# bitlayer-org/tap-stark

Measured on AMD Instinct MI355X. Metric: trace cells/sec (proofs/sec alongside), 2^20x64 BabyBear trace, higher is better.
Workload: dtype u32

## Files before the change

tap-stark_amd/csrc/context.cpp:

```cpp
#include <errno.h>
#include <stdio.h>
#include <time.h>
#include <stdlib.h>
#include "context.hpp"

#include <string.h>

#include "kernels.hpp"

namespace ts {

static bool poison_knob(uint32_t* word) {
    const char* e = getenv("TS_POOL_POISON");
    if (!e || !*e) return false;
    char* end = nullptr;
    errno = 0;
    const unsigned long v = strtoul(e, &end, 0);
    TS_REQUIRE(errno == 0 && end != e && *end == 0 && e[0] != '-' && v <= 0xFFFFFFFFul, TS_ERR_INVALID,
               "TS_POOL_POISON is not a 32-bit word (decimal, 0x hex or 0 octal)");
    *word = (uint32_t)v;
    return true;
}

Context::Context(int dev) : device(dev) {
    pool_debug = getenv("TS_POOL_DEBUG") != nullptr;
    poison_on = poison_knob(&poison_word);
    int count = 0;
    hipError_t e = hipGetDeviceCount(&count);
    if (e != hipSuccess || count == 0)
        throw Error(TS_ERR_HIP, "no HIP device available: the tap-stark HIP path has no CPU fallback");
    TS_REQUIRE(dev >= 0 && dev < count, TS_ERR_INVALID, "device index out of range");
    TS_HIP(hipSetDevice(dev));
    hipDeviceProp_t prop;
    TS_HIP(hipGetDeviceProperties(&prop, dev));
    num_cus = prop.multiProcessorCount;
    max_lds_per_block = prop.sharedMemPerBlock;
    arch_name = prop.gcnArchName;
    arch_name = arch_name.substr(0, arch_name.find(':'));
    TS_HIP(hipStreamCreateWithFlags(&stream, hipStreamNonBlocking));
}

Context::~Context() {
    (void)hipSetDevice(device);
    if (stream) (void)hipStreamSynchronize(stream);
    if (d_twiddle_fwd) (void)hipFree(d_twiddle_fwd);
    if (d_twiddle_inv) (void)hipFree(d_twiddle_inv);
    for (auto& t : scale_tables) (void)hipFree(t.d);
    for (auto& t : sel_tables)
        if (t.d) (void)hipFree(t.d);
    if (d_ticket) (void)hipFree(d_ticket);
    for (auto& kv : free_blocks) (void)hipFree(kv.second);
    for (auto& kv : live_blocks) (void)hipFree(kv.first);
    if (h_pinned) (void)hipHostFree(h_pinned);
    if (h_mailbox) (void)hipHostFree(h_mailbox);
    if (h_mailbox_big) (void)hipHostFree(h_mailbox_big);
    if (h_arena) (void)hipHostFree(h_arena);
    if (stream) (void)hipStreamDestroy(stream);
}

static size_t round_block(size_t bytes) {
    if (bytes < 512) return 512;
    if (bytes < (1u << 20)) {
        size_t r = 512;
        while (r < bytes) r <<= 1;
        return r;
    }
    const size_t g = 1u << 20;
    return (bytes + g - 1) / g * g;
}

void* Context::alloc(size_t bytes) {
    const size_t sz = round_block(bytes);
    auto it = free_blocks.find(sz);
    void* p = nullptr;
    if (it != free_blocks.end()) {
        p = it->second;
        free_blocks.erase(it);
    } else {
        TS_HIP(hipSetDevice(device));
        if (pool_debug) {
            struct timespec ts_;
            clock_gettime(CLOCK_MONOTONIC, &ts_);
            fprintf(stderr, "[ts pool %p t=%.3f ms] hipMalloc %zu KiB (reserved %zu MiB)\n", (void*)this,
                    ts_.tv_sec * 1e3 + ts_.tv_nsec * 1e-6, sz >> 10, bytes_reserved >> 20);
        }
        hipError_t e = hipMalloc(&p, sz);
        if (e != hipSuccess) {
            release_cache();
            e = hipMalloc(&p, sz);
        }
        if (e != hipSuccess) {
            (void)hipGetLastError();
            throw Error(TS_ERR_OOM, "device allocation failed");
        }
        bytes_reserved += sz;
    }
    live_blocks[p] = sz;
    if (poison_on) poison(p, sz);
    return p;
}

void Context::poison(void* p, size_t bytes) {
    TS_HIP(hipSetDevice(device));
    TS_HIP(hipMemsetD32Async((hipDeviceptr_t)p, (int)poison_word, bytes / 4, stream));
    TS_HIP(hipStreamSynchronize(stream));
    poison_fills++;
}

void Context::free(void* p) {
    if (!p) return;
    auto it = live_blocks.find(p);
    if (it == live_blocks.end()) return;
    free_blocks.emplace(it->second, p);
    live_blocks.erase(it);
}

void Context::release_cache() {
    if (stream) (void)hipStreamSynchronize(stream);
    for (auto& kv : free_blocks) {
        (void)hipFree(kv.second);
        bytes_reserved -= kv.first;
    }
    free_blocks.clear();
}

uint32_t* Context::ticket() {
    if (!d_ticket) {
        TS_HIP(hipMalloc((void**)&d_ticket, 64 * 17));
        TS_HIP(hipMemsetAsync(d_ticket, 0, 64 * 17, stream));
    }
    return d_ticket;
}

const void* Context::stage(const void* src, size_t bytes) {
    const size_t need = (bytes + 63) & ~(size_t)63;
    if (need > h_arena_bytes / 2) {
        sync();
        if (h_arena) (void)hipHostFree(h_arena);
        h_arena = nullptr;
        size_t sz = 1 << 20;
        while (sz / 2 < need) sz <<= 1;
        TS_HIP(hipHostMalloc((void**)&h_arena, sz, hipHostMallocDefault));
        h_arena_bytes = sz;
        h_arena_off = 0;
    }
    if (h_arena_off + need > h_arena_bytes) {
        sync();
        h_arena_off = 0;
    }
    void* p = h_arena + h_arena_off;
    memcpy(p, src, bytes);
    h_arena_off += need;
    return p;
}

void Context::sync_point(void* host, size_t bytes) {
    if (replay_mode == 2 && replay_pos < replay_log.size() && replay_log[replay_pos].size() == bytes) {
        memcpy(host, replay_log[replay_pos++].data(), bytes);
        return;
    }
    sync();
    if (replay_mode == 1) replay_log.emplace_back((const char*)host, (const char*)host + bytes);
}
void Context::d2h_point(void* host_dst, const void* dev_src, size_t bytes) {
    if (replay_mode == 2 && replay_pos < replay_log.size() && replay_log[replay_pos].size() == bytes) {
        memcpy(host_dst, replay_log[replay_pos++].data(), bytes);
        return;
    }
    if (bytes) TS_HIP(hipMemcpyAsync(host_dst, dev_src, bytes, hipMemcpyDeviceToHost, stream));
    sync();
    if (replay_mode == 1) replay_log.emplace_back((const char*)host_dst, (const char*)host_dst + bytes);
}

uint32_t* Context::mailbox(size_t words) {
    constexpr size_t WORDS = 16384;
    if (words > WORDS / 4) {
        if (words > h_mailbox_big_words) {
            sync();
            if (h_mailbox_big) (void)hipHostFree(h_mailbox_big);
            h_mailbox_big = nullptr;
            h_mailbox_big_words = 0;
            TS_HIP(hipHostMalloc((void**)&h_mailbox_big, words * 4, hipHostMallocDefault));
            h_mailbox_big_words = words;
        }
        return h_mailbox_big;
    }
    if (!h_mailbox) TS_HIP(hipHostMalloc((void**)&h_mailbox, WORDS * 4, hipHostMallocDefault));
    const size_t need = (words + 15) & ~(size_t)15;
    if (mailbox_off + need > WORDS) mailbox_off = 0;
    uint32_t* p = h_mailbox + mailbox_off;
    mailbox_off += need;
    return p;
}

void* Context::pinned(size_t bytes) {
    if (bytes > h_pinned_bytes) {
        if (h_pinned) {
            sync();
            (void)hipHostFree(h_pinned);
        }
        size_t sz = 1 << 16;
        while (sz < bytes) sz <<= 1;
        TS_HIP(hipHostMalloc(&h_pinned, sz, hipHostMallocDefault));
        h_pinned_bytes = sz;
    }
    return h_pinned;
}

std::map<std::string, std::pair<uint64_t, double>> Context::take_kernel_timings() {
    std::map<std::string, std::pair<uint64_t, double>> out;
    sync();
    for (auto& ev : kernel_events) {
        float ms = 0;
        (void)hipEventElapsedTime(&ms, ev.e0, ev.e1);
        auto& slot = out[ev.name];
        slot.first += 1;
        slot.second += ms;
        (void)hipEventDestroy(ev.e0);
        (void)hipEventDestroy(ev.e1);
    }
    kernel_events.clear();
    return out;
}

void Context::ensure_twiddles(unsigned log_size) {
    if (log_size <= twiddle_log && d_twiddle_fwd) return;
    TS_REQUIRE(log_size <= 27, TS_ERR_INVALID, "two-adicity of BabyBear is 27");
    sync();
    if (d_twiddle_fwd) (void)hipFree(d_twiddle_fwd);
    if (d_twiddle_inv) (void)hipFree(d_twiddle_inv);
    d_twiddle_fwd = d_twiddle_inv = nullptr;
    const size_t n = (size_t)1 << log_size;
    TS_HIP(hipMalloc((void**)&d_twiddle_fwd, n * 4));
    TS_HIP(hipMalloc((void**)&d_twiddle_inv, n * 4));
    if (poison_on) {
        poison(d_twiddle_fwd, n * 4);
        poison(d_twiddle_inv, n * 4);
    }
    twiddle_log = log_size;
    launch_build_twiddles(*this, d_twiddle_fwd, d_twiddle_inv, log_size);
}

}
```

tap-stark_amd/csrc/context.hpp:

```cpp
#pragma once
#include <hip/hip_runtime.h>
#include <stdint.h>

#include <map>
#include <stdexcept>
#include <string>
#include <vector>

#include "bb.hpp"

namespace ts {

struct Error : std::runtime_error {
    int code;
    Error(int c, const std::string& m) : std::runtime_error(m), code(c) {}
};

struct FinalPolyNotConstant : Error {
    explicit FinalPolyNotConstant(const std::string& m) : Error(5 , m) {}
};

enum : int {
    TS_OK = 0,
    TS_ERR_INVALID = 1,
    TS_ERR_HIP = 2,
    TS_ERR_OOM = 3,
    TS_ERR_UNSUPPORTED = 4,
    TS_ERR_INVARIANT = 5,
    TS_ERR_BUFFER = 6,
    TS_ERR_COMM = 7,
};

#define TS_HIP(expr)                                                                        \
    do {                                                                                    \
        hipError_t _e = (expr);                                                             \
        if (_e != hipSuccess)                                                               \
            throw ts::Error(ts::TS_ERR_HIP, std::string(#expr) + ": " + hipGetErrorString(_e)); \
    } while (0)

#define TS_REQUIRE(cond, code, msg)                   \
    do {                                              \
        if (!(cond)) throw ts::Error((code), (msg));  \
    } while (0)

struct Context {
    int device = 0;
    hipStream_t stream = nullptr;
    std::string last_error;
    int num_cus = 256;
    size_t max_lds_per_block = 64 * 1024;
    std::string arch_name;

    std::multimap<size_t, void*> free_blocks;
    std::map<void*, size_t> live_blocks;
    size_t bytes_reserved = 0;
    bool pool_debug = false;
    bool poison_on = false;
    uint32_t poison_word = 0;
    uint64_t poison_fills = 0;
    void poison(void* p, size_t bytes);

    uint32_t* d_twiddle_fwd = nullptr;
    uint32_t* d_twiddle_inv = nullptr;
    unsigned twiddle_log = 0;

    struct ScaleTable {
        unsigned log_n, log_blowup;
        uint32_t shift;
        uint32_t* d;
        size_t words;
        uint64_t last_use;
    };
    std::vector<ScaleTable> scale_tables;
    uint64_t scale_clock = 0;
    struct SelTable {
        uint32_t* d = nullptr;
        unsigned log_n = ~0u, log_qd = ~0u;
        uint32_t shift = 0;
        uint64_t last_use = 0;
    };
    SelTable sel_tables[2];
    uint64_t sel_clock = 0;

    uint32_t* d_ticket = nullptr;
    uint32_t* ticket();

    unsigned lde_pass_mask = 7;

    uint32_t* h_mailbox = nullptr;
    size_t mailbox_off = 0;
    uint32_t* h_mailbox_big = nullptr;
    size_t h_mailbox_big_words = 0;
    uint32_t* mailbox(size_t words);

    void* h_pinned = nullptr;
    size_t h_pinned_bytes = 0;
    char* h_arena = nullptr;
    size_t h_arena_bytes = 0, h_arena_off = 0;
    const void* stage(const void* src, size_t bytes);

    bool timing = false;
    std::vector<std::pair<std::string, float>> stage_ms;

    struct KernelEvent {
        const char* name;
        hipEvent_t e0, e1;
    };
    bool kernel_timing = false;
    std::vector<KernelEvent> kernel_events;
    std::map<std::string, std::pair<uint64_t, double>> take_kernel_timings();

    uint64_t pow_hints_accepted = 0, pow_hints_rejected = 0, pow_host_grinds = 0;
    uint64_t local_quotient_fallbacks = 0;

    explicit Context(int dev);
    ~Context();
    Context(const Context&) = delete;

    void* alloc(size_t bytes);
    void free(void* p);
    template <class T>
    T* alloc_n(size_t n) { return static_cast<T*>(alloc(n * sizeof(T))); }
    void release_cache();

    int replay_mode = 0;
    size_t replay_pos = 0;
    std::vector<std::vector<char>> replay_log;
    void sync_point(void* host, size_t bytes);
    void d2h_point(void* host_dst, const void* dev_src, size_t bytes);
    void* pinned(size_t bytes);
    void ensure_twiddles(unsigned log_size);
    void sync() { TS_HIP(hipStreamSynchronize(stream)); }
};

template <class T>
struct DevBuf {
    Context* ctx = nullptr;
    T* p = nullptr;
    size_t n = 0;
    DevBuf() = default;
    DevBuf(Context* c, size_t count) : ctx(c), p(c->alloc_n<T>(count)), n(count) {}
    DevBuf(const DevBuf&) = delete;
    DevBuf& operator=(const DevBuf&) = delete;
    DevBuf(DevBuf&& o) noexcept : ctx(o.ctx), p(o.p), n(o.n) { o.p = nullptr; }
    DevBuf& operator=(DevBuf&& o) noexcept {
        if (this != &o) {
            reset();
            ctx = o.ctx; p = o.p; n = o.n; o.p = nullptr;
        }
        return *this;
    }
    ~DevBuf() { reset(); }
    void reset() {
        if (p) ctx->free(p);
        p = nullptr;
    }
};

struct KernelTimer {
    Context* ctx;
    Context::KernelEvent ev;
    bool on;
    KernelTimer(Context* c, const char* name) : ctx(c), on(c->kernel_timing) {
        if (on) {
            ev.name = name;
            (void)hipEventCreate(&ev.e0);
            (void)hipEventCreate(&ev.e1);
            (void)hipEventRecord(ev.e0, ctx->stream);
        }
    }
    ~KernelTimer() {
        if (on) {
            (void)hipEventRecord(ev.e1, ctx->stream);
            ctx->kernel_events.push_back(ev);
        }
    }
};

#define TS_LAUNCH_NAMED(ctx, name, kernel, grid, block, lds, ...)                   \
    do {                                                                            \
        ts::KernelTimer _kt(&(ctx), name);                                          \
        hipLaunchKernelGGL(kernel, grid, block, lds, (ctx).stream, __VA_ARGS__);    \
    } while (0)
#define TS_LAUNCH(ctx, kernel, ...) TS_LAUNCH_NAMED(ctx, #kernel, kernel, __VA_ARGS__)

struct StageTimer {
    Context* ctx;
    const char* name;
    hipEvent_t e0 = nullptr, e1 = nullptr;
    StageTimer(Context* c, const char* n) : ctx(c), name(n) {
        if (ctx->timing) {
            (void)hipEventCreate(&e0);
            (void)hipEventCreate(&e1);
            (void)hipEventRecord(e0, ctx->stream);
        }
    }
    ~StageTimer() {
        if (ctx->timing && e0) {
            (void)hipEventRecord(e1, ctx->stream);
            (void)hipEventSynchronize(e1);
            float ms = 0;
            (void)hipEventElapsedTime(&ms, e0, e1);
            ctx->stage_ms.emplace_back(name, ms);
            (void)hipEventDestroy(e0);
            (void)hipEventDestroy(e1);
        }
    }
};

}
```

tap-stark_amd/csrc/host.hpp:

```cpp
#pragma once
#include <stdint.h>

#include <algorithm>
#include <functional>
#include <memory>
#include <vector>

#include "air.hpp"
#include "bb.hpp"
#include "chal_dev.hpp"
#include "context.hpp"
#include "kernels.hpp"

namespace ts {

class BfChallenger {
public:
    enum Permutation { Blake3Permutation = 0, TestReversePermutation = 1 };
    BfChallenger(int permutation, bool sample_ext)
        : permutation_(permutation), sample_ext_(sample_ext) {}

    void observe(uint32_t word);
    void observe_commitment(const uint32_t d[8]);
    uint32_t sample_base();
    Ef sample_ext();
    Ef sample();
    uint64_t sample_bits(unsigned bits);
    bool check_witness(unsigned bits, uint32_t witness);
    uint32_t grind(unsigned bits);
    void export_state(uint32_t out[34]) const;
    void export_dev(DevChallenger& d) const;
    void import_dev(const DevChallenger& d);

private:
    void duplexing();
    uint32_t pop();
    uint32_t state_[16] = {0};
    uint32_t in_[8] = {0};
    int n_in_ = 0;
    uint32_t out_[8] = {0};
    int n_out_ = 0;
    int permutation_;
    bool sample_ext_;
};

struct FriConfig {
    uint32_t log_blowup = 1;
    uint32_t num_queries = 1;
    uint32_t proof_of_work_bits = 0;
    uint32_t blowup() const { return 1u << log_blowup; }
};

struct DeviceMatrix {
    enum Layout { ROW_MAJOR, COL_MAJOR_BITREV };
    DevBuf<uint32_t> buf;
    uint64_t height = 0;
    uint32_t width = 0;
    Layout layout = ROW_MAJOR;
};

struct PcsData {
    std::vector<DevBuf<uint32_t>> lde_storage;
    std::vector<ColMat> ldes;
    unsigned log_height = 0;
    DevBuf<uint32_t> tree;
    DevBuf<const uint32_t*> col_table;
    bool col_table_uploaded = false;
    uint32_t root[8] = {0};
    LeafMats leaf_mats() const;
    LeafMats leaf_mats_with_table(Context& ctx);
};
std::vector<const uint32_t*> column_pointers(const std::vector<ColMat>& ldes, uint64_t height = 0);
bool columns_as_one_matrix(const std::vector<ColMat>& ldes, uint64_t height, uint32_t max_width, ColMat& one);

unsigned log2_strict(uint64_t n);

void mmcs_commit(Context& ctx, PcsData& data);

class TwoAdicFriPcs {
public:
    TwoAdicFriPcs(Context& ctx, FriConfig fri) : ctx_(ctx), fri_(fri) {}
    const FriConfig& fri() const { return fri_; }
    Context& ctx() const { return ctx_; }

    std::unique_ptr<PcsData> commit(std::vector<DeviceMatrix>& evals,
                                    const std::vector<uint32_t>& domain_shifts, bool build_tree = true,
                                    bool keep_row_major = false);

    std::vector<DeviceMatrix> quotient_chunks(const PcsData& trace_data, const AirProgram& air,
                                              const std::vector<uint32_t>& public_values, Ef alpha,
                                              const PcsData* preprocessed = nullptr, const PcsData* aux = nullptr);

    DevBuf<Ef> open_reduce(const PcsData& trace_data, const PcsData& quotient_data, Ef zeta,
                           Ef batch_alpha, std::vector<Ef>& opened_values, const PcsData* preprocessed = nullptr,
                           const PcsData* aux = nullptr);

    struct Slab {
        uint64_t row0 = 0, rows = 0;
        uint32_t beta0 = 0;
    };
    std::vector<DeviceMatrix> quotient_chunks_slab(const ColMat& lde_slab, unsigned log_n, const Slab& slab,
                                                   const AirProgram& air,
                                                   const std::vector<uint32_t>& public_values, Ef alpha,
                                                   uint32_t domain_shift = GENERATOR,
                                                   const ColMat* prep_lde = nullptr, const ColMat* aux_lde = nullptr);
    DevBuf<Ef> open_reduce_slab(const PcsData& trace_data, const PcsData& quotient_data, unsigned log_N,
                                const Slab& slab, Ef zeta, Ef batch_alpha, std::vector<Ef>& opened_values,
                                const PcsData* preprocessed = nullptr, const PcsData* aux = nullptr);

    struct OpenRound {
        const PcsData* data = nullptr;
        std::vector<std::vector<Ef>> points;
    };
    std::vector<uint32_t> open(const std::vector<OpenRound>& rounds, BfChallenger& challenger,
                               std::vector<Ef>& opened_values);

    void fri_prove(std::vector<DevBuf<Ef>>& inputs, const std::vector<unsigned>& log_lens,
                   BfChallenger& challenger, const std::vector<const PcsData*>& input_rounds,
                   std::vector<uint32_t>& pf, bool pass_through = false);

    void open_batch(const PcsData& d, uint64_t index, std::vector<uint32_t>& rows,
                    std::vector<uint32_t>& path);

private:
    Context& ctx_;
    FriConfig fri_;
};

std::vector<uint32_t> prove(TwoAdicFriPcs& pcs, const AirProgram& air, BfChallenger& challenger,
                            DeviceMatrix trace, const std::vector<uint32_t>& public_values,
                            const PcsData* preprocessed = nullptr, uint32_t proof_version = 1);
using AuxSource = std::function<DeviceMatrix(const DeviceMatrix& trace, const uint32_t* challenges, uint32_t* exposed)>;
std::vector<uint32_t> prove_aux(TwoAdicFriPcs& pcs, const AirProgram& air, BfChallenger& challenger,
                                DeviceMatrix trace, const std::vector<uint32_t>& public_values,
                                const AuxSource& aux_source);
std::vector<uint32_t> prove_pre_aux(TwoAdicFriPcs& pcs, const AirProgram& air, BfChallenger& challenger,
                                    DeviceMatrix trace, const std::vector<uint32_t>& public_values,
                                    const PcsData* preprocessed, const AuxSource& aux_source);
void check_third_matrix(const PcsData& aux, const AirProgram& air, uint64_t lde_height);
void check_preprocessed_key(const PcsData& key, const AirProgram& air, uint64_t lde_height);

struct Comm {
    int rank = 0, world = 1;
    std::function<void(const void* send, void* recv, size_t bytes_per_rank, hipStream_t stream)> all_gather;
    std::function<void(void* buf, size_t bytes, int root, hipStream_t stream)> broadcast;
};
struct ShardOptions {
    unsigned min_local_log = 12;
    bool trace_replicated = false;
    bool local_quotient = false;
};
std::vector<uint32_t> prove_sharded(TwoAdicFriPcs& pcs, const Comm& comm, const AirProgram& air,
                                    BfChallenger& challenger, DeviceMatrix trace_rows,
                                    const std::vector<uint32_t>& public_values, const ShardOptions& opt);

struct TapLocks {
    const uint8_t* bytes = nullptr;
    const uint64_t* offsets = nullptr;
    size_t n_scripts = 0;
};
std::vector<uint32_t> prove_tap(TwoAdicFriPcs& pcs, const AirProgram& air, BfChallenger& challenger,
                                DeviceMatrix trace, const std::vector<uint32_t>& public_values,
                                const TapLocks& locks, const Comm* comm = nullptr);
int verify_tap(const FriConfig& fri, const AirProgram& air, BfChallenger& challenger,
               const uint32_t* proof, size_t n_words, const std::vector<uint32_t>& public_values,
               const TapLocks& locks);
bool tap_verify_words(const TapLocks& locks, size_t first, uint32_t n_evals, uint32_t u32_size,
                      uint64_t index, const uint32_t* values, const uint32_t* path_words, size_t depth,
                      const uint32_t root_words[8]);

int verify(const FriConfig& fri, const AirProgram& air, BfChallenger& challenger,
           const uint32_t* proof, size_t n_words, const std::vector<uint32_t>& public_values);
int verify_pre(const FriConfig& fri, const AirProgram& air, BfChallenger& challenger, const uint32_t* preprocessed_root,
               const uint32_t* proof, size_t n_words, const std::vector<uint32_t>& public_values);
int verify_aux(const FriConfig& fri, const AirProgram& air, BfChallenger& challenger, const uint32_t* proof,
               size_t n_words, const std::vector<uint32_t>& public_values, std::vector<uint32_t>& exposed);
int verify_pre_aux(const FriConfig& fri, const AirProgram& air, BfChallenger& challenger,
                   const uint32_t* preprocessed_root, const uint32_t* proof, size_t n_words,
                   const std::vector<uint32_t>& public_values, std::vector<uint32_t>& exposed);

struct PcsMatClaim {
    unsigned log_height;
    uint32_t width;
    std::vector<Ef> points;
    std::vector<std::vector<Ef>> values;
};
struct PcsRoundClaim {
    const uint32_t* root = nullptr;
    std::vector<PcsMatClaim> mats;
};
int pcs_verify(const FriConfig& fri, BfChallenger& challenger, const std::vector<PcsRoundClaim>& rounds,
               const uint32_t* fri_proof, size_t n_words);
int fri_verify_pass_through(const FriConfig& fri, BfChallenger& challenger, const uint32_t* fri_proof,
                            size_t n_words);

bool tspf_to_postcard(const uint32_t* words, size_t n_words, std::vector<uint8_t>& out);
bool postcard_to_tspf(const uint8_t* bytes, size_t n_bytes, std::vector<uint32_t>& out, int want_version = 0);

}
```

tap-stark_amd/csrc/kernels.hpp:

```cpp
#pragma once
#include <stdint.h>

#include "bb.hpp"
#include "context.hpp"
#include "ntt_plan.hpp"

namespace ts {

struct ColMat {
    uint32_t* d = nullptr;
    uint64_t height = 0;
    uint32_t width = 0;
    uint64_t col_stride = 0;
};

void launch_build_twiddles(Context& ctx, uint32_t* W, uint32_t* Winv, unsigned log_size);
void launch_build_shift_tables(Context& ctx, uint32_t* lo, uint32_t* hi, uint32_t n_hi,
                               uint32_t n_cosets, uint32_t shift_mont, unsigned log_N,
                               unsigned log_blowup, uint32_t scale_mont);
const uint32_t* coset_scale_table(Context& ctx, unsigned log_n, unsigned log_blowup, uint32_t shift);
void launch_transpose_bitrev(Context& ctx, const uint32_t* src, uint32_t* dst, unsigned log_n,
                             uint32_t w, uint64_t dst_col_stride, uint32_t src_width = 0);
bool launch_transpose_bitrev_r16(Context& ctx, const uint32_t* src, uint32_t* dst, unsigned log_n, uint32_t w,
                                 uint64_t dst_col_stride, uint32_t src_width = 0);
void launch_transpose_plain(Context& ctx, const uint32_t* src, uint32_t* dst, uint64_t n, uint32_t w,
                            uint64_t dst_col_stride);
void launch_transpose_to_row_major(Context& ctx, const uint32_t* src, uint64_t col_stride,
                                   uint32_t* dst, uint64_t h, uint32_t w);
void launch_transpose_unbitrev(Context& ctx, const uint32_t* src, uint64_t col_stride, uint32_t* dst,
                               unsigned log_h, uint32_t w);
void coset_lde(Context& ctx, uint32_t* evals, uint64_t in_col_stride, uint32_t ncols, unsigned log_n,
               unsigned log_blowup, uint32_t shift, uint32_t* out, uint64_t out_col_stride,
               uint32_t beta0 = 0, uint32_t n_beta = 0, bool first_round_done = false,
               uint32_t* evals2 = nullptr, uint32_t shift2 = 0, uint32_t gw = 0, bool stage_timers = true);

constexpr uint32_t LDE_NO_OWN = 0xffffffffu;
int lde_own_coset_used(unsigned log_n, unsigned log_blowup, uint32_t shift);

inline void ntt_require_shape(const NttPlan& p, uint32_t ncols, uint64_t stride_a, uint64_t stride_b, bool lde) {
    if (const char* why = ntt_plan_refusal(p, ncols, stride_a, stride_b, lde)) throw Error(TS_ERR_INVALID, why);
}
void launch_contig_inverse(Context& ctx, const NttPlan& p, uint32_t* data, uint64_t col_stride, uint32_t ncols,
                           bool first_round_done = false, uint32_t* data2 = nullptr, uint32_t gw = 0xffffffffu);
void launch_contig_forward(Context& ctx, const NttPlan& p, uint32_t* data, uint64_t col_stride, uint32_t ncols,
                           uint32_t n_blocks, uint32_t gw = 0xffffffffu, uint32_t own_a = LDE_NO_OWN,
                           uint32_t own_b = LDE_NO_OWN);

void dft_columns(Context& ctx, uint32_t* cols, uint64_t col_stride, uint32_t ncols, unsigned log_n, bool inverse,
                 uint32_t shift);
void dft_batch(Context& ctx, const uint32_t* in, uint32_t* out, unsigned log_n, uint32_t w, bool inverse,
               uint32_t shift);
void coset_lde_batch(Context& ctx, const uint32_t* in, uint32_t* out, unsigned log_n, uint32_t w, unsigned added_bits,
                     uint32_t shift, bool bit_reversed);
void launch_bit_reverse_rows(Context& ctx, const uint32_t* src, uint32_t* dst, unsigned log_h, uint32_t w);

constexpr int MAX_BATCH_MATS = 64;
struct LeafMats {
    const uint32_t* d[MAX_BATCH_MATS];
    uint64_t col_stride[MAX_BATCH_MATS];
    uint32_t width[MAX_BATCH_MATS];
    uint8_t row_shift[MAX_BATCH_MATS];
    uint32_t n_mats;
    uint32_t total_width;
    const uint32_t* const* cols;
};
void launch_leaf_hash(Context& ctx, const LeafMats& mats, uint64_t height, uint32_t* digests);
void launch_leaf_hash_ef_pairs(Context& ctx, const uint32_t* vec, uint64_t n_rows, uint32_t* digests);
struct DevChallenger;
bool launch_merkle_levels(Context& ctx, uint32_t* tree, unsigned log_leaves,
                          DevChallenger* ch = nullptr, uint32_t* root_out = nullptr,
                          Ef* beta_out = nullptr);
void launch_merkle_tree_from(Context& ctx, uint32_t* tree, unsigned log_leaves, unsigned first_level,
                             DevChallenger* ch, uint32_t* root_out, Ef* beta_out);
bool leaf_tree_enabled(unsigned log_leaves);
void launch_commit_tree(Context& ctx, const LeafMats& mats, unsigned log_leaves, uint32_t* tree,
                        uint32_t* root_out = nullptr);
void launch_shard_top(Context& ctx, const uint32_t* subroots, uint32_t G, uint32_t* top,
                      DevChallenger* ch, uint32_t* root_out, Ef* beta_out);
void launch_merkle_one_level(Context& ctx, const uint32_t* children, uint32_t* parents,
                             uint64_t n_parents);
void launch_merkle_inject(Context& ctx, uint32_t* nodes, const uint32_t* inj, uint64_t n);
inline uint64_t merkle_level_offset(unsigned log_leaves, unsigned level) {
    uint64_t off = 0;
    for (unsigned l = 0; l < level; l++) off += (uint64_t)1 << (log_leaves - l);
    return off;
}
inline uint64_t merkle_total_digests(unsigned log_leaves) { return ((uint64_t)2 << log_leaves) - 1; }

struct AirProgram;
const uint32_t* selector_table(Context& ctx, unsigned log_n, unsigned log_qd, uint32_t shift);
constexpr int MAX_QUOTIENT_CHUNKS = 64;
struct QuotOut {
    uint32_t* chunk[MAX_QUOTIENT_CHUNKS];
};
void launch_quotient(Context& ctx, const AirProgram& air, const ColMat& trace_lde, unsigned log_n,
                     unsigned log_qd, const uint32_t* d_consts_mont, const uint32_t* d_alpha_pows_mont,
                     const QuotOut& out, uint64_t row_begin = 0, uint64_t row_end = 0,
                     uint32_t shift = GENERATOR, const ColMat* prep_lde = nullptr, const ColMat* aux_lde = nullptr);
void launch_chunk_mix(Context& ctx, uint32_t* const* d_chunk_ptrs, uint32_t qd, uint64_t rows, uint64_t col_stride,
                      const uint32_t* d_mix_mont);

void launch_check_constraints(Context& ctx, const AirProgram& air, const uint32_t* trace_row_major,
                              uint64_t n, const uint32_t* d_consts_mont,
                              unsigned long long* d_violation, const uint32_t* prep_row_major = nullptr,
                              const uint32_t* aux_row_major = nullptr);

void launch_bary_weights(Context& ctx, unsigned log_n, const Ef* points_mont, uint32_t n_points,
                         Ef* out, uint32_t coset_gen = 0);
struct BaryPending {
    DevBuf<uint32_t> partial[4];
    uint32_t* out[4] = {nullptr, nullptr, nullptr, nullptr};
    uint32_t n_blocks[4] = {0, 0, 0, 0}, n_words[4] = {0, 0, 0, 0};
    uint32_t n = 0, capacity = 2;
};
void launch_bary_dots(Context& ctx, const ColMat& m, unsigned log_n, const Ef* weights,
                      uint32_t n_points, Ef* out, BaryPending* pending = nullptr);
void launch_bary_finish(Context& ctx, BaryPending& pending);
struct ReduceArgs {
    Ef z_mont[2];
    Ef off_mont[2];
    Ef rys[2];
    uint32_t n_points;
    uint32_t accumulate;
};
void launch_reduce(Context& ctx, const ColMat& m, unsigned log_h, const uint32_t* d_alpha_pows_mont,
                   const ReduceArgs& args, Ef* ro);
struct FusedReduceArgs {
    Ef z_mont[2];
    Ef off_t[2];
    Ef k0, k1;
    const uint32_t* chunk_w;
    const uint32_t* chunk[MAX_QUOTIENT_CHUNKS];
    uint64_t chunk_stride;
    uint32_t n_chunks;
    uint64_t row0, rows;
};
void launch_reduce_fused(Context& ctx, const ColMat& trace, unsigned log_h,
                         const uint32_t* d_alpha_pows_mont, const FusedReduceArgs& args, Ef* ro,
                         const ColMat* prep = nullptr, const Ef* prep_off_mont = nullptr,
                         const ColMat* aux = nullptr, const Ef* aux_off_mont = nullptr);
void launch_reduce_low(Context& ctx, const ColMat& trace, unsigned log_n, const uint32_t* d_alpha_pows_mont,
                       const FusedReduceArgs& args, const Ef* weights, uint32_t* out);
void launch_ef_interleave(Context& ctx, const uint32_t* cols, uint64_t col_stride, uint64_t rows, Ef* out);

void launch_fri_fold(Context& ctx, const Ef* in, uint64_t h, Ef beta_canonical, Ef* out,
                     uint32_t* next_digests);
void launch_fri_fold_dev(Context& ctx, const Ef* in, uint64_t h, const Ef* d_beta, Ef* out,
                         uint32_t* next_digests, uint64_t h_global = 0, uint64_t row0 = 0);
struct FriRoundLaunch {
    const Ef* prev = nullptr;
    const Ef* d_beta_prev = nullptr;
    Ef* cur = nullptr;
    uint64_t h = 0;
    uint32_t* tree = nullptr;
    DevChallenger* ch = nullptr;
    uint32_t* root_out = nullptr;
    Ef* beta_out = nullptr;
    uint64_t h_global = 0, row0 = 0;
};
void launch_fri_commit_round(Context& ctx, const FriRoundLaunch& r);
constexpr int FRI_TAIL_LOG = 10;
constexpr uint32_t FRI_POW_NONE = 0xffffffffu;
void launch_fri_tail(Context& ctx, const Ef* in, uint32_t L0, uint32_t blowup, DevChallenger* ch,
                     Ef* tail_vecs, uint32_t* tail_trees, uint32_t* roots_out, Ef* betas_out,
                     Ef* final_out, uint32_t pow_bits = 0, uint32_t* pow_out = nullptr,
                     const Ef* beta_in = nullptr);
void launch_vec_add(Context& ctx, Ef* acc, const Ef* other, uint64_t n);
struct FriGatherDesc {
    const uint32_t* vec;
    const uint32_t* tree;
    uint32_t log_leaves;
    uint32_t shift;
    uint64_t out_vals;
    uint64_t out_path;
};
struct RowGatherJob {
    LeafMats mats;
    uint32_t shift;
    uint32_t pad;
    uint64_t out;
};
void launch_gather_queries(Context& ctx, const RowGatherJob* d_rows, uint32_t n_rows, uint32_t max_row_width,
                           const FriGatherDesc* d_descs, uint32_t n_descs, uint32_t max_log_leaves,
                           const uint32_t* d_indices, uint32_t n_idx, uint32_t* out);

double alu_ceiling(Context& ctx, int kind);
double bench_stage(Context& ctx, int stage, unsigned log_n, uint32_t width, unsigned log_blowup, uint32_t reps);

void launch_trace_fibonacci(Context& ctx, uint32_t* out, uint32_t a, uint32_t b, uint64_t n);
void launch_trace_synth_mul(Context& ctx, uint32_t* out, uint64_t n, uint32_t width, uint64_t seed);
void launch_trace_synth_ext(Context& ctx, uint32_t* out, uint64_t n, uint32_t width, uint64_t seed);

enum : uint8_t { COL_U32 = 0, COL_U16 = 1, COL_U8 = 2, COL_MONTY32 = 3, COL_MONTY31 = 4 };
struct IngestPlan {
    bool planar = false;
    uint64_t height = 0;
    uint32_t width = 0;
    uint64_t stride = 0;
    uint64_t bytes = 0;
    int uniform4 = -1;
    std::vector<uint64_t> table;
};
IngestPlan ingest_plan(const uint8_t* kinds, uint32_t n_kinds, bool planar, uint64_t row_stride, uint64_t height,
                       uint32_t width);
void launch_ingest(Context& ctx, const IngestPlan& plan, const uint8_t* src, uint32_t* out);
void launch_scale_words(Context& ctx, const uint32_t* in, uint32_t* out, uint64_t n, uint32_t mult);
uint32_t monty_ingest_factor(uint32_t kind);

}
```

tap-stark_amd/csrc/open.hip:

```cpp
#include "kernels.hpp"

namespace ts {

__device__ __forceinline__ uint32_t root_bitrev(const uint32_t* __restrict__ W, unsigned L, uint64_t r) {
    if (L == 0) return R_MOD_P;
    uint32_t w = W[((uint64_t)1 << (L - 1)) + (r >> 1)];
    return (r & 1) ? neg(w) : w;
}

constexpr int BW_ROWS = 4;

__global__ void __launch_bounds__(256)
k_bary_weights(unsigned log_n, const uint32_t* __restrict__ W, uint32_t gen_mont, Ef z0, Ef z1,
               uint32_t n_points, Ef* __restrict__ out) {
    const uint64_t n = 1ull << log_n;
    const uint64_t t0 = ((uint64_t)blockIdx.x * blockDim.x + threadIdx.x) * BW_ROWS;
    if (t0 >= n) return;
    Ef num[2 * BW_ROWS];
    uint32_t nrm[2 * BW_ROWS], pre[2 * BW_ROWS], xs[BW_ROWS];
    uint32_t run = R_MOD_P;
#pragma unroll
    for (int k = 0; k < BW_ROWS; k++) {
        const bool ok = t0 + k < n;
        uint32_t x = ok ? mont_mul(gen_mont, root_bitrev(W, log_n, t0 + k)) : R_MOD_P;
        xs[k] = x;
#pragma unroll
        for (int p = 0; p < 2; p++) {
            const Ef z = p == 0 ? z0 : z1;
            Ef u = Ef{{sub(z.c[0], x), z.c[1], z.c[2], z.c[3]}};
            if (p < (int)n_points && ok) {
                ef_inv_parts(u, num[2 * k + p], nrm[2 * k + p]);
            } else {
                num[2 * k + p] = ef_zero();
                nrm[2 * k + p] = R_MOD_P;
            }
            pre[2 * k + p] = run;
            run = mont_mul(run, nrm[2 * k + p]);
        }
    }
    uint32_t inv = mont_inv(run);
#pragma unroll
    for (int j = 2 * BW_ROWS - 1; j >= 0; j--) {
        uint32_t ninv = mont_mul(inv, pre[j]);
        inv = mont_mul(inv, nrm[j]);
        const int k = j >> 1, p = j & 1;
        if (p < (int)n_points && t0 + k < n)
            out[(uint64_t)p * n + t0 + k] = ef_mul_base(num[j], mont_mul(ninv, xs[k]));
    }
}

void launch_bary_weights(Context& ctx, unsigned log_n, const Ef* points_mont, uint32_t n_points,
                         Ef* out, uint32_t coset_gen) {
    TS_REQUIRE(n_points >= 1 && n_points <= 2, TS_ERR_INVALID, "bary_weights: 1 or 2 points");
    ctx.ensure_twiddles(log_n == 0 ? 1 : log_n);
    const uint64_t threads = (((uint64_t)1 << log_n) + BW_ROWS - 1) / BW_ROWS;
    Ef z0 = points_mont[0], z1 = n_points > 1 ? points_mont[1] : points_mont[0];
    TS_LAUNCH(ctx, k_bary_weights, dim3((unsigned)((threads + 255) / 256)), dim3(256), 0, log_n,
              ctx.d_twiddle_fwd, to_mont(coset_gen ? coset_gen : GENERATOR), z0, z1, n_points, out);
    TS_HIP(hipGetLastError());
}

template <int NP, int COLS>
__global__ void __launch_bounds__(256)
k_bary_dots(const uint32_t* __restrict__ m, uint64_t col_stride, uint32_t width, unsigned log_n,
            const Ef* __restrict__ weights, uint32_t* __restrict__ partial, uint32_t rows_per_block) {
    constexpr int RS = 64 / COLS;
    constexpr int TR = 16 * 4 * RS;
    constexpr int PER_THREAD = COLS * TR / 256;
    __shared__ uint32_t tile[16 * 257];
    __shared__ uint32_t wts[TR][NP * 4];
    __shared__ uint32_t red[4 * RS][COLS][NP * 4];
    const uint64_t n = 1ull << log_n;
    const uint32_t c0 = blockIdx.y * COLS;
    const uint32_t lane = threadIdx.x & 63, wv = threadIdx.x >> 6;
    const uint32_t cl = lane % COLS, rs = lane / COLS;
    const uint32_t sub = wv * RS + rs;
    const uint64_t row_begin = (uint64_t)blockIdx.x * rows_per_block;
    const uint64_t row_end = row_begin + rows_per_block < n ? row_begin + rows_per_block : n;
    uint64_t acc[NP * 4];
#pragma unroll
    for (int j = 0; j < NP * 4; j++) acc[j] = 0;
    for (uint64_t row0 = row_begin; row0 < row_end; row0 += TR) {
        uint32_t v[PER_THREAD];
#pragma unroll
        for (int k = 0; k < PER_THREAD; k++) {
            const uint32_t e = threadIdx.x + (uint32_t)k * 256;
            const uint32_t c = c0 + e / TR;
            const uint64_t t = row0 + e % TR;
            v[k] = (c < width && t < row_end) ? m[(uint64_t)c * col_stride + t] : 0u;
        }
        for (uint32_t e = threadIdx.x; e < (uint32_t)(TR * NP); e += 256) {
            const uint32_t p = e / TR, tt = e % TR;
            const uint64_t t = row0 + tt;
            Ef w = ef_zero();
            if (t < row_end) w = weights[(uint64_t)p * n + t];
            wts[tt][p * 4 + 0] = w.c[0];
            wts[tt][p * 4 + 1] = w.c[1];
            wts[tt][p * 4 + 2] = w.c[2];
            wts[tt][p * 4 + 3] = w.c[3];
        }
#pragma unroll
        for (int k = 0; k < PER_THREAD; k++) {
            const uint32_t e = threadIdx.x + (uint32_t)k * 256;
            const uint32_t t = e % TR;
            tile[(t & 15) * 257 + (t >> 4) * COLS + e / TR] = v[k];
        }
        __syncthreads();
#pragma unroll
        for (int rr = 0; rr < 16; rr++) {
            const uint32_t tt = sub * 16 + rr;
            const uint32_t x = tile[rr * 257 + sub * COLS + cl];
#pragma unroll
            for (int j = 0; j < NP * 4; j++) acc[j] = lazy_mac(acc[j], x, wts[tt][j]);
            if (rr & 1) {
#pragma unroll
                for (int j = 0; j < NP * 4; j++) acc[j] = lazy_fix(acc[j]);
            }
        }
        __syncthreads();
    }
#pragma unroll
    for (int j = 0; j < NP * 4; j++) red[sub][cl][j] = lazy_finish(acc[j]);
    __syncthreads();
    for (uint32_t idx = threadIdx.x; idx < (uint32_t)(COLS * NP * 4); idx += 256) {
        const uint32_t c = idx / (NP * 4), j = idx % (NP * 4);
        uint32_t sum = 0;
#pragma unroll
        for (int q = 0; q < 4 * RS; q++) sum = add(sum, red[q][c][j]);
        if (c0 + c < width)
            partial[((uint64_t)blockIdx.x * width + c0 + c) * (NP * 4) + j] = sum;
    }
}

struct BaryFinishJob {
    const uint32_t* partial;
    uint32_t* out;
    uint32_t n_blocks, n_words;
};
__device__ __forceinline__ void bary_finish_group(const uint32_t* __restrict__ partial, uint32_t* __restrict__ out,
                                                  uint32_t n_blocks, uint32_t n_words, uint32_t group) {
    __shared__ uint32_t red[4][4];
    const uint32_t j = group * 4 + (threadIdx.x & 3);
    uint32_t v = 0;
    if (j < n_words) {
        uint32_t b = threadIdx.x >> 2;
        for (; b + 7 * 64 < n_blocks; b += 8 * 64) {
            uint32_t x[8];
#pragma unroll
            for (int k = 0; k < 8; k++) x[k] = partial[(uint64_t)(b + 64 * k) * n_words + j];
#pragma unroll
            for (int k = 0; k < 8; k++) v = add(v, x[k]);
        }
        for (; b < n_blocks; b += 64) v = add(v, partial[(uint64_t)b * n_words + j]);
    }
#pragma unroll
    for (int off = 32; off >= 4; off >>= 1) v = add(v, __shfl_down(v, off, 64));
    const uint32_t lane = threadIdx.x & 63, wv = threadIdx.x >> 6;
    if (lane < 4) red[wv][lane] = v;
    __syncthreads();
    if (threadIdx.x < 4 && j < n_words)
        out[j] = add(add(red[0][threadIdx.x], red[1][threadIdx.x]),
                     add(red[2][threadIdx.x], red[3][threadIdx.x]));
}
__global__ void __launch_bounds__(256)
k_bary_finish(BaryFinishJob j0, BaryFinishJob j1, uint32_t g0) {
    const bool first = blockIdx.x < g0;
    bary_finish_group(first ? j0.partial : j1.partial, first ? j0.out : j1.out, first ? j0.n_blocks : j1.n_blocks,
                      first ? j0.n_words : j1.n_words, first ? blockIdx.x : blockIdx.x - g0);
}
__global__ void __launch_bounds__(256)
k_bary_finish3(BaryFinishJob j0, BaryFinishJob j1, BaryFinishJob j2, uint32_t g0, uint32_t g1) {
    const BaryFinishJob j = blockIdx.x < g0 ? j0 : blockIdx.x < g0 + g1 ? j1 : j2;
    bary_finish_group(j.partial, j.out, j.n_blocks, j.n_words,
                      blockIdx.x < g0 ? blockIdx.x : blockIdx.x < g0 + g1 ? blockIdx.x - g0 : blockIdx.x - g0 - g1);
}

__global__ void __launch_bounds__(256)
k_bary_finish4(BaryFinishJob j0, BaryFinishJob j1, BaryFinishJob j2, BaryFinishJob j3, uint32_t g0, uint32_t g1,
               uint32_t g2) {
    const uint32_t b = blockIdx.x;
    const BaryFinishJob j = b < g0 ? j0 : b < g0 + g1 ? j1 : b < g0 + g1 + g2 ? j2 : j3;
    bary_finish_group(j.partial, j.out, j.n_blocks, j.n_words,
                      b < g0 ? b : b < g0 + g1 ? b - g0 : b < g0 + g1 + g2 ? b - g0 - g1 : b - g0 - g1 - g2);
}

void launch_bary_finish(Context& ctx, BaryPending& pend) {
    if (pend.n == 0) return;
    BaryFinishJob j[4] = {{nullptr, nullptr, 0, 0}, {nullptr, nullptr, 0, 0}, {nullptr, nullptr, 0, 0},
                          {nullptr, nullptr, 0, 0}};
    uint32_t g[4] = {0, 0, 0, 0};
    for (uint32_t i = 0; i < pend.n; i++) {
        j[i] = BaryFinishJob{pend.partial[i].p, pend.out[i], pend.n_blocks[i], pend.n_words[i]};
        g[i] = (pend.n_words[i] + 3) / 4;
    }
    if (pend.n == 4)
        TS_LAUNCH(ctx, k_bary_finish4, dim3(g[0] + g[1] + g[2] + g[3]), dim3(256), 0, j[0], j[1], j[2], j[3], g[0], g[1],
                  g[2]);
    else if (pend.n == 3)
        TS_LAUNCH(ctx, k_bary_finish3, dim3(g[0] + g[1] + g[2]), dim3(256), 0, j[0], j[1], j[2], g[0], g[1]);
    else
        TS_LAUNCH(ctx, k_bary_finish, dim3(g[0] + g[1]), dim3(256), 0, j[0], j[1], g[0]);
    TS_HIP(hipGetLastError());
    for (uint32_t i = 0; i < pend.n; i++) pend.partial[i].reset();
    pend.n = 0;
}

void launch_bary_dots(Context& ctx, const ColMat& m, unsigned log_n, const Ef* weights,
                      uint32_t n_points, Ef* out, BaryPending* pending) {
    const uint64_t n = 1ull << log_n;
    const bool narrow = m.width <= 8;
    const uint32_t tr = narrow ? 512 : 64;
    uint32_t n_blocks = (uint32_t)((n + tr - 1) / tr);
    if (n_blocks > 2048) n_blocks = 2048;
    uint32_t rows_per_block = (uint32_t)(((n + n_blocks - 1) / n_blocks + tr - 1) / tr * tr);
    n_blocks = (uint32_t)((n + rows_per_block - 1) / rows_per_block);
    const uint32_t n_words = m.width * n_points * 4;
    DevBuf<uint32_t> partial(&ctx, (size_t)n_blocks * n_words);
    const uint32_t* md = m.d;
    if (narrow) {
        dim3 grid(n_blocks, (m.width + 7) / 8);
        if (n_points == 2)
            TS_LAUNCH(ctx, (k_bary_dots<2, 8>), grid, dim3(256), 0, md, m.col_stride, m.width, log_n,
                      weights, partial.p, rows_per_block);
        else
            TS_LAUNCH(ctx, (k_bary_dots<1, 8>), grid, dim3(256), 0, md, m.col_stride, m.width, log_n,
                      weights, partial.p, rows_per_block);
    } else {
        dim3 grid(n_blocks, (m.width + 63) / 64);
        if (n_points == 2)
            TS_LAUNCH(ctx, (k_bary_dots<2, 64>), grid, dim3(256), 0, md, m.col_stride, m.width, log_n,
                      weights, partial.p, rows_per_block);
        else
            TS_LAUNCH(ctx, (k_bary_dots<1, 64>), grid, dim3(256), 0, md, m.col_stride, m.width, log_n,
                      weights, partial.p, rows_per_block);
    }
    TS_HIP(hipGetLastError());
    BaryPending own;
    BaryPending& pend = pending ? *pending : own;
    if (pend.n == pend.capacity) launch_bary_finish(ctx, pend);
    pend.partial[pend.n] = std::move(partial);
    pend.out[pend.n] = reinterpret_cast<uint32_t*>(out);
    pend.n_blocks[pend.n] = n_blocks;
    pend.n_words[pend.n] = n_words;
    pend.n++;
    if (!pending) launch_bary_finish(ctx, pend);
}

__device__ __forceinline__ void row_dot_acc(uint64_t (&acc)[4], const uint32_t* __restrict__ m,
                                            uint64_t col_stride, uint32_t width, uint64_t X,
                                            const uint32_t* __restrict__ weights) {
    uint64_t a0 = acc[0], a1 = acc[1], a2 = acc[2], a3 = acc[3];
    constexpr int B = 8;
    const uint32_t* col = m + X;
    uint32_t i = 0;
    for (; i + B <= width; i += B) {
        uint32_t v[B];
#pragma unroll
        for (int k = 0; k < B; k++) v[k] = col[(uint64_t)(i + k) * col_stride];
#pragma unroll
        for (int k = 0; k < B; k++) {
            const uint32_t* ap = weights + 4 * (i + k);
            a0 = lazy_mac(a0, v[k], ap[0]);
            a1 = lazy_mac(a1, v[k], ap[1]);
            a2 = lazy_mac(a2, v[k], ap[2]);
            a3 = lazy_mac(a3, v[k], ap[3]);
            if (k & 1) {
                a0 = lazy_fix(a0);
                a1 = lazy_fix(a1);
                a2 = lazy_fix(a2);
                a3 = lazy_fix(a3);
            }
        }
    }
    if (i < width) {
        uint32_t v[B];
#pragma unroll
        for (int k = 0; k < B; k++) v[k] = i + k < width ? col[(uint64_t)(i + k) * col_stride] : 0u;
#pragma unroll
        for (int k = 0; k < B; k++) {
            if (i + k < width) {
                const uint32_t* ap = weights + 4 * (i + k);
                a0 = lazy_mac(a0, v[k], ap[0]);
                a1 = lazy_mac(a1, v[k], ap[1]);
                a2 = lazy_mac(a2, v[k], ap[2]);
                a3 = lazy_mac(a3, v[k], ap[3]);
            }
            if (k & 1) {
                a0 = lazy_fix(a0);
                a1 = lazy_fix(a1);
                a2 = lazy_fix(a2);
                a3 = lazy_fix(a3);
            }
        }
    }
    acc[0] = a0; acc[1] = a1; acc[2] = a2; acc[3] = a3;
}
__device__ __forceinline__ Ef row_dot_alpha(const uint32_t* __restrict__ m, uint64_t col_stride,
                                            uint32_t width, uint64_t X,
                                            const uint32_t* __restrict__ alpha_pows) {
    uint64_t acc[4] = {0, 0, 0, 0};
    row_dot_acc(acc, m, col_stride, width, X, alpha_pows);
    return Ef{{lazy_finish(acc[0]), lazy_finish(acc[1]), lazy_finish(acc[2]), lazy_finish(acc[3])}};
}

template <int NP>
__device__ __forceinline__ void inv_denoms(uint32_t x_mont, const Ef* z_mont, Ef* out) {
    Ef num[NP];
    uint32_t nrm[NP];
#pragma unroll
    for (int p = 0; p < NP; p++) {
        const Ef z = z_mont[p];
        Ef u = Ef{{sub(x_mont, z.c[0]), neg(z.c[1]), neg(z.c[2]), neg(z.c[3])}};
        ef_inv_parts(u, num[p], nrm[p]);
    }
    if (NP == 2) {
        uint32_t inv = mont_inv(mont_mul(nrm[0], nrm[NP - 1]));
        out[0] = ef_mul_base(num[0], mont_mul(inv, nrm[NP - 1]));
        out[NP - 1] = ef_mul_base(num[NP - 1], mont_mul(inv, nrm[0]));
    } else {
        out[0] = ef_mul_base(num[0], mont_inv(nrm[0]));
    }
}

template <int NP>
__global__ void __launch_bounds__(256)
k_reduce(const uint32_t* __restrict__ m, uint64_t col_stride, uint32_t width, unsigned log_h,
         const uint32_t* __restrict__ W, uint32_t gen_mont, const uint32_t* __restrict__ alpha_pows,
         ReduceArgs args, Ef* __restrict__ ro) {
    const uint64_t h = 1ull << log_h;
    const uint64_t X = (uint64_t)blockIdx.x * blockDim.x + threadIdx.x;
    if (X >= h) return;
    const Ef S = row_dot_alpha(m, col_stride, width, X, alpha_pows);
    const uint32_t x = mont_mul(gen_mont, root_bitrev(W, log_h, X));
    Ef inv_d[NP];
    inv_denoms<NP>(x, args.z_mont, inv_d);
    Ef acc = args.accumulate ? ro[X] : ef_zero();
#pragma unroll
    for (int p = 0; p < NP; p++) {
        Ef t = ef_mul(ef_sub(S, args.rys[p]), args.off_mont[p]);
        acc = ef_add(acc, ef_mul(t, inv_d[p]));
    }
    ro[X] = acc;
}

void launch_reduce(Context& ctx, const ColMat& m, unsigned log_h, const uint32_t* d_alpha_pows_mont,
                   const ReduceArgs& args, Ef* ro) {
    TS_REQUIRE(args.n_points >= 1 && args.n_points <= 2, TS_ERR_INVALID, "reduce: 1 or 2 points");
    ctx.ensure_twiddles(log_h == 0 ? 1 : log_h);
    const uint64_t h = 1ull << log_h;
    dim3 grid((unsigned)((h + 255) / 256));
    if (args.n_points == 2)
        TS_LAUNCH(ctx, k_reduce<2>, grid, dim3(256), 0, (const uint32_t*)m.d, m.col_stride, m.width,
                  log_h, (const uint32_t*)ctx.d_twiddle_fwd, to_mont(GENERATOR), d_alpha_pows_mont, args,
                  ro);
    else
        TS_LAUNCH(ctx, k_reduce<1>, grid, dim3(256), 0, (const uint32_t*)m.d, m.col_stride, m.width,
                  log_h, (const uint32_t*)ctx.d_twiddle_fwd, to_mont(GENERATOR), d_alpha_pows_mont, args,
                  ro);
    TS_HIP(hipGetLastError());
}

__global__ void __launch_bounds__(256)
k_reduce_fused(const uint32_t* __restrict__ trace, uint64_t trace_stride, uint32_t width,
               unsigned log_h, const uint32_t* __restrict__ W, uint32_t gen_mont,
               const uint32_t* __restrict__ alpha_pows, FusedReduceArgs a, Ef* __restrict__ ro) {
    const uint64_t X = (uint64_t)blockIdx.x * blockDim.x + threadIdx.x;
    if (X >= a.rows) return;
    const Ef St = row_dot_alpha(trace, trace_stride, width, X, alpha_pows);
    const uint32_t x = mont_mul(gen_mont, root_bitrev(W, log_h, a.row0 + X));
    Ef inv_d[2];
    inv_denoms<2>(x, a.z_mont, inv_d);
    uint64_t acc[4] = {0, 0, 0, 0};
    uint32_t c = 0;
    for (; c + 2 <= a.n_chunks; c += 2) {
        uint32_t v[8];
#pragma unroll
        for (int k = 0; k < 8; k++) v[k] = a.chunk[c + (k >> 2)][(uint64_t)(k & 3) * a.chunk_stride + X];
        const uint32_t* ap = a.chunk_w + 16 * c;
#pragma unroll
        for (int k = 0; k < 8; k++) {
#pragma unroll
            for (int j = 0; j < 4; j++) acc[j] = lazy_mac(acc[j], v[k], ap[4 * k + j]);
            if (k & 1) {
#pragma unroll
                for (int j = 0; j < 4; j++) acc[j] = lazy_fix(acc[j]);
            }
        }
    }
    for (; c < a.n_chunks; c++) row_dot_acc(acc, a.chunk[c], a.chunk_stride, 4, X, a.chunk_w + 16 * c);
    const Ef D{{lazy_finish(acc[0]), lazy_finish(acc[1]), lazy_finish(acc[2]), lazy_finish(acc[3])}};
    const Ef g0 = ef_sub(ef_add(ef_mul(St, a.off_t[0]), D), a.k0);
    const Ef g1 = ef_sub(ef_mul(St, a.off_t[1]), a.k1);
    const Ef r = ef_add(ef_mul(g0, inv_d[0]), ef_mul(g1, inv_d[1]));
    *reinterpret_cast<uint4*>(ro + X) = make_uint4(r.c[0], r.c[1], r.c[2], r.c[3]);
}

struct PrepReduceArgs {
    const uint32_t* prep;
    uint64_t stride;
    uint32_t width;
    Ef off_p[2];
};
__global__ void __launch_bounds__(256)
k_reduce_fused_pre(const uint32_t* __restrict__ trace, uint64_t trace_stride, uint32_t width,
               unsigned log_h, const uint32_t* __restrict__ W, uint32_t gen_mont,
               const uint32_t* __restrict__ alpha_pows, FusedReduceArgs a, PrepReduceArgs pa,
               Ef* __restrict__ ro) {
    const uint64_t X = (uint64_t)blockIdx.x * blockDim.x + threadIdx.x;
    if (X >= a.rows) return;
    const Ef St = row_dot_alpha(trace, trace_stride, width, X, alpha_pows);
    const uint32_t x = mont_mul(gen_mont, root_bitrev(W, log_h, a.row0 + X));
    Ef inv_d[2];
    inv_denoms<2>(x, a.z_mont, inv_d);
    uint64_t acc[4] = {0, 0, 0, 0};
    uint32_t c = 0;
    for (; c + 2 <= a.n_chunks; c += 2) {
        uint32_t v[8];
#pragma unroll
        for (int k = 0; k < 8; k++) v[k] = a.chunk[c + (k >> 2)][(uint64_t)(k & 3) * a.chunk_stride + X];
        const uint32_t* ap = a.chunk_w + 16 * c;
#pragma unroll
        for (int k = 0; k < 8; k++) {
#pragma unroll
            for (int j = 0; j < 4; j++) acc[j] = lazy_mac(acc[j], v[k], ap[4 * k + j]);
            if (k & 1) {
#pragma unroll
                for (int j = 0; j < 4; j++) acc[j] = lazy_fix(acc[j]);
            }
        }
    }
    for (; c < a.n_chunks; c++) row_dot_acc(acc, a.chunk[c], a.chunk_stride, 4, X, a.chunk_w + 16 * c);
    const Ef D{{lazy_finish(acc[0]), lazy_finish(acc[1]), lazy_finish(acc[2]), lazy_finish(acc[3])}};
    const Ef Sp = row_dot_alpha(pa.prep, pa.stride, pa.width, X, alpha_pows);
    const Ef g0 = ef_sub(ef_add(ef_add(ef_mul(St, a.off_t[0]), ef_mul(Sp, pa.off_p[0])), D), a.k0);
    const Ef g1 = ef_sub(ef_add(ef_mul(St, a.off_t[1]), ef_mul(Sp, pa.off_p[1])), a.k1);
    const Ef r = ef_add(ef_mul(g0, inv_d[0]), ef_mul(g1, inv_d[1]));
    *reinterpret_cast<uint4*>(ro + X) = make_uint4(r.c[0], r.c[1], r.c[2], r.c[3]);
}

struct PrepAuxReduceArgs {
    const uint32_t* prep;
    const uint32_t* aux;
    uint64_t prep_stride, aux_stride;
    uint32_t prep_width, aux_width;
    Ef off_p[2];
    Ef off_a[2];
};
__global__ void __launch_bounds__(256)
k_reduce_fused_pre_aux(const uint32_t* __restrict__ trace, uint64_t trace_stride, uint32_t width,
                       unsigned log_h, const uint32_t* __restrict__ W, uint32_t gen_mont,
                       const uint32_t* __restrict__ alpha_pows, FusedReduceArgs a, PrepAuxReduceArgs pa,
                       Ef* __restrict__ ro) {
    const uint64_t X = (uint64_t)blockIdx.x * blockDim.x + threadIdx.x;
    if (X >= a.rows) return;
    const Ef St = row_dot_alpha(trace, trace_stride, width, X, alpha_pows);
    const uint32_t x = mont_mul(gen_mont, root_bitrev(W, log_h, a.row0 + X));
    Ef inv_d[2];
    inv_denoms<2>(x, a.z_mont, inv_d);
    uint64_t acc[4] = {0, 0, 0, 0};
    uint32_t c = 0;
    for (; c + 2 <= a.n_chunks; c += 2) {
        uint32_t v[8];
#pragma unroll
        for (int k = 0; k < 8; k++) v[k] = a.chunk[c + (k >> 2)][(uint64_t)(k & 3) * a.chunk_stride + X];
        const uint32_t* ap = a.chunk_w + 16 * c;
#pragma unroll
        for (int k = 0; k < 8; k++) {
#pragma unroll
            for (int j = 0; j < 4; j++) acc[j] = lazy_mac(acc[j], v[k], ap[4 * k + j]);
            if (k & 1) {
#pragma unroll
                for (int j = 0; j < 4; j++) acc[j] = lazy_fix(acc[j]);
            }
        }
    }
    for (; c < a.n_chunks; c++) row_dot_acc(acc, a.chunk[c], a.chunk_stride, 4, X, a.chunk_w + 16 * c);
    const Ef D{{lazy_finish(acc[0]), lazy_finish(acc[1]), lazy_finish(acc[2]), lazy_finish(acc[3])}};
    const Ef Sp = row_dot_alpha(pa.prep, pa.prep_stride, pa.prep_width, X, alpha_pows);
    const Ef Sa = row_dot_alpha(pa.aux, pa.aux_stride, pa.aux_width, X, alpha_pows);
    const Ef g0 = ef_sub(ef_add(ef_add(ef_add(ef_mul(St, a.off_t[0]), ef_mul(Sp, pa.off_p[0])), ef_mul(Sa, pa.off_a[0])), D),
                         a.k0);
    const Ef g1 = ef_sub(ef_add(ef_add(ef_mul(St, a.off_t[1]), ef_mul(Sp, pa.off_p[1])), ef_mul(Sa, pa.off_a[1])), a.k1);
    const Ef r = ef_add(ef_mul(g0, inv_d[0]), ef_mul(g1, inv_d[1]));
    *reinterpret_cast<uint4*>(ro + X) = make_uint4(r.c[0], r.c[1], r.c[2], r.c[3]);
}

void launch_reduce_fused(Context& ctx, const ColMat& trace, unsigned log_h,
                         const uint32_t* d_alpha_pows_mont, const FusedReduceArgs& args, Ef* ro,
                         const ColMat* prep, const Ef* prep_off_mont, const ColMat* aux, const Ef* aux_off_mont) {
    TS_REQUIRE(args.n_chunks <= (uint32_t)MAX_QUOTIENT_CHUNKS, TS_ERR_INVALID, "reduce_fused: too many chunks");
    ctx.ensure_twiddles(log_h == 0 ? 1 : log_h);
    FusedReduceArgs a = args;
    if (a.rows == 0) {
        a.row0 = 0;
        a.rows = 1ull << log_h;
    }
    TS_REQUIRE(a.row0 + a.rows <= (1ull << log_h), TS_ERR_INVALID, "reduce_fused: row range");
    TS_REQUIRE(!aux || prep, TS_ERR_INVARIANT, "reduce_fused: a third matrix without a second");
    if (aux) {
        for (const ColMat* m : {prep, aux})
            TS_REQUIRE(m->d && a.row0 == 0 && m->height == a.rows && m->col_stride >= a.rows, TS_ERR_INVALID,
                       "reduce_fused: preprocessed or aux matrix shape");
        TS_REQUIRE(prep_off_mont && aux_off_mont, TS_ERR_INVALID, "reduce_fused: missing offsets");
        const PrepAuxReduceArgs pa{prep->d, aux->d, prep->col_stride, aux->col_stride, prep->width, aux->width,
                                   {prep_off_mont[0], prep_off_mont[1]}, {aux_off_mont[0], aux_off_mont[1]}};
        TS_LAUNCH(ctx, k_reduce_fused_pre_aux, dim3((unsigned)((a.rows + 255) / 256)), dim3(256), 0,
                  (const uint32_t*)trace.d, trace.col_stride, trace.width, log_h,
                  (const uint32_t*)ctx.d_twiddle_fwd, to_mont(GENERATOR), d_alpha_pows_mont, a, pa, ro);
        TS_HIP(hipGetLastError());
        return;
    }
    if (prep) {
        TS_REQUIRE(prep_off_mont && prep->d && a.row0 == 0 && prep->height == a.rows && prep->col_stride >= a.rows,
                   TS_ERR_INVALID, "reduce_fused: preprocessed matrix shape");
        const PrepReduceArgs pa{prep->d, prep->col_stride, prep->width, {prep_off_mont[0], prep_off_mont[1]}};
        TS_LAUNCH(ctx, k_reduce_fused_pre, dim3((unsigned)((a.rows + 255) / 256)), dim3(256), 0,
                  (const uint32_t*)trace.d, trace.col_stride, trace.width, log_h,
                  (const uint32_t*)ctx.d_twiddle_fwd, to_mont(GENERATOR), d_alpha_pows_mont, a, pa, ro);
        TS_HIP(hipGetLastError());
        return;
    }
    TS_LAUNCH(ctx, k_reduce_fused, dim3((unsigned)((a.rows + 255) / 256)), dim3(256), 0,
              (const uint32_t*)trace.d, trace.col_stride, trace.width, log_h,
              (const uint32_t*)ctx.d_twiddle_fwd, to_mont(GENERATOR), d_alpha_pows_mont, a, ro);
    TS_HIP(hipGetLastError());
}

__device__ __forceinline__ Ef chunk_dot(const FusedReduceArgs& a, uint64_t X) {
    uint64_t acc[4] = {0, 0, 0, 0};
    uint32_t c = 0;
    for (; c + 2 <= a.n_chunks; c += 2) {
        uint32_t v[8];
#pragma unroll
        for (int k = 0; k < 8; k++) v[k] = a.chunk[c + (k >> 2)][(uint64_t)(k & 3) * a.chunk_stride + X];
        const uint32_t* ap = a.chunk_w + 16 * c;
#pragma unroll
        for (int k = 0; k < 8; k++) {
#pragma unroll
            for (int j = 0; j < 4; j++) acc[j] = lazy_mac(acc[j], v[k], ap[4 * k + j]);
            if (k & 1) {
#pragma unroll
                for (int j = 0; j < 4; j++) acc[j] = lazy_fix(acc[j]);
            }
        }
    }
    for (; c < a.n_chunks; c++) row_dot_acc(acc, a.chunk[c], a.chunk_stride, 4, X, a.chunk_w + 16 * c);
    return Ef{{lazy_finish(acc[0]), lazy_finish(acc[1]), lazy_finish(acc[2]), lazy_finish(acc[3])}};
}

__global__ void __launch_bounds__(256)
k_reduce_low(const uint32_t* __restrict__ trace, uint64_t trace_stride, uint32_t width, unsigned log_n,
             const uint32_t* __restrict__ Winv, uint32_t gen_inv_mont, const uint32_t* __restrict__ alpha_pows,
             FusedReduceArgs a, const Ef* __restrict__ weights, uint32_t* __restrict__ out) {
    const uint64_t n = 1ull << log_n;
    const uint64_t t = (uint64_t)blockIdx.x * blockDim.x + threadIdx.x;
    if (t >= n) return;
    const Ef St = row_dot_alpha(trace, trace_stride, width, t, alpha_pows);
    const Ef D = chunk_dot(a, t);
    const uint32_t nxi = neg(mont_mul(gen_inv_mont, root_bitrev(Winv, log_n, t)));
    const Ef inv_d0 = ef_mul_base(weights[t], nxi), inv_d1 = ef_mul_base(weights[n + t], nxi);
    const Ef g0 = ef_sub(ef_add(ef_mul(St, a.off_t[0]), D), a.k0);
    const Ef g1 = ef_sub(ef_mul(St, a.off_t[1]), a.k1);
    const Ef r = ef_add(ef_mul(g0, inv_d0), ef_mul(g1, inv_d1));
#pragma unroll
    for (int k = 0; k < 4; k++) out[(uint64_t)k * n + t] = r.c[k];
}

void launch_reduce_low(Context& ctx, const ColMat& trace, unsigned log_n, const uint32_t* d_alpha_pows_mont,
                       const FusedReduceArgs& args, const Ef* weights, uint32_t* out) {
    TS_REQUIRE(args.n_chunks <= (uint32_t)MAX_QUOTIENT_CHUNKS, TS_ERR_INVALID, "reduce_low: too many chunks");
    const uint64_t n = 1ull << log_n;
    TS_REQUIRE(args.row0 == 0 && trace.height >= n && trace.col_stride >= n && args.chunk_stride >= n, TS_ERR_INVALID,
               "reduce_low: the matrices must start with the low coset");
    ctx.ensure_twiddles(log_n == 0 ? 1 : log_n);
    TS_LAUNCH(ctx, k_reduce_low, dim3((unsigned)((n + 255) / 256)), dim3(256), 0, (const uint32_t*)trace.d,
              trace.col_stride, trace.width, log_n, (const uint32_t*)ctx.d_twiddle_inv,
              to_mont(inv_canon(GENERATOR)), d_alpha_pows_mont, args, weights, out);
    TS_HIP(hipGetLastError());
}

__global__ void __launch_bounds__(256)
k_ef_interleave(const uint32_t* __restrict__ cols, uint64_t col_stride, uint64_t rows, Ef* __restrict__ out) {
    const uint64_t X = (uint64_t)blockIdx.x * blockDim.x + threadIdx.x;
    if (X >= rows) return;
    *reinterpret_cast<uint4*>(out + X) = make_uint4(cols[X], cols[col_stride + X], cols[2 * col_stride + X],
                                                    cols[3 * col_stride + X]);
}

void launch_ef_interleave(Context& ctx, const uint32_t* cols, uint64_t col_stride, uint64_t rows, Ef* out) {
    TS_REQUIRE(col_stride >= rows, TS_ERR_INVALID, "ef_interleave: column stride below the row count");
    TS_LAUNCH(ctx, k_ef_interleave, dim3((unsigned)((rows + 255) / 256)), dim3(256), 0, cols, col_stride, rows, out);
    TS_HIP(hipGetLastError());
}

}
```

tap-stark_amd/csrc/prover.cpp:

```cpp
#include <string.h>

#include <algorithm>

#include "prover_internal.hpp"

namespace ts {

void mmcs_commit(Context& ctx, PcsData& data) {
    const unsigned log_H = data.log_height;
    const uint64_t N = 1ull << log_H;
    bool uniform = true;
    for (auto& cm : data.ldes) uniform = uniform && cm.height == N;
    {
        StageTimer t(&ctx, "merkle_commit");
        data.tree = DevBuf<uint32_t>(&ctx, merkle_total_digests(log_H) * 8);
        std::vector<const uint32_t*> cols;
        struct Group { uint64_t height; size_t first; uint32_t total; };
        std::vector<Group> groups;
        for (unsigned lh = log_H + 1; lh-- > 0;) {
            const std::vector<const uint32_t*> gc = column_pointers(data.ldes, 1ull << lh);
            if (!gc.empty()) groups.push_back(Group{1ull << lh, cols.size(), (uint32_t)gc.size()});
            cols.insert(cols.end(), gc.begin(), gc.end());
        }
        data.col_table = DevBuf<const uint32_t*>(&ctx, cols.size());
        data.col_table_uploaded = false;
        auto group_mats = [&](const Group& g) {
            LeafMats lm;
            memset(&lm, 0, sizeof lm);
            lm.cols = data.col_table.p + g.first;
            lm.total_width = g.total;
            ColMat one;
            if (columns_as_one_matrix(data.ldes, g.height, 256, one)) {
                lm.n_mats = 1;
                lm.d[0] = one.d;
                lm.col_stride[0] = one.col_stride;
                lm.width[0] = one.width;
            } else if (!data.col_table_uploaded) {
                h2d(ctx, data.col_table.p, cols.data(), cols.size() * sizeof(const uint32_t*));
                data.col_table_uploaded = true;
            }
            return lm;
        };
        auto group_leaves = [&](const Group& g, uint32_t* digests) {
            launch_leaf_hash(ctx, group_mats(g), g.height, digests);
        };
        uint32_t* mail = nullptr;
        if (uniform) {
            if (log_H >= 1) mail = ctx.mailbox(8);
            launch_commit_tree(ctx, group_mats(groups[0]), log_H, data.tree.p, mail);
        } else {
            group_leaves(groups[0], data.tree.p);
            DevBuf<uint32_t> inj(&ctx, 8 * (N / 2));
            size_t gi = 1;
            for (unsigned l = 1; l <= log_H; l++) {
                uint32_t* children = data.tree.p + 8 * merkle_level_offset(log_H, l - 1);
                uint32_t* parents = data.tree.p + 8 * merkle_level_offset(log_H, l);
                const uint64_t n_par = N >> l;
                launch_merkle_one_level(ctx, children, parents, n_par);
                if (gi < groups.size() && groups[gi].height == n_par) {
                    group_leaves(groups[gi], inj.p);
                    launch_merkle_inject(ctx, parents, inj.p, n_par);
                    gi++;
                }
            }
        }
        if (mail) {
            ctx.sync_point(mail, 32);
            memcpy(data.root, mail, 32);
        } else {
            d2h_sync(ctx, data.root, data.tree.p + 8 * (merkle_total_digests(log_H) - 1), 32);
        }
    }
}

std::unique_ptr<PcsData> TwoAdicFriPcs::commit(std::vector<DeviceMatrix>& evals,
                                               const std::vector<uint32_t>& domain_shifts, bool build_tree,
                                               bool keep_row_major) {
    auto data = std::make_unique<PcsData>();
    lde_stage(ctx_, fri_, evals, domain_shifts, 0, 0, true, *data, keep_row_major);
    if (build_tree) mmcs_commit(ctx_, *data);
    return data;
}

void check_preprocessed_key(const PcsData& key, const AirProgram& air, uint64_t lde_height) {
    TS_REQUIRE(key.ldes.size() == 1, TS_ERR_INVALID, "preprocessed key: exactly one committed matrix expected");
    TS_REQUIRE(air.second_width() > 0 && key.ldes[0].width == air.second_width(), TS_ERR_INVALID,
               "preprocessed key: width differs from the AIR's preprocessed width");
    TS_REQUIRE(key.ldes[0].height == lde_height, TS_ERR_INVALID,
               "preprocessed key: LDE height is not the trace height << log_blowup");
}

void check_third_matrix(const PcsData& aux, const AirProgram& air, uint64_t lde_height) {
    TS_REQUIRE(aux.ldes.size() == 1, TS_ERR_INVALID, "aux data: exactly one committed matrix expected");
    TS_REQUIRE(air.has_third() && aux.ldes[0].width == air.third_width(), TS_ERR_INVALID,
               "aux data: width differs from the AIR's aux width");
    TS_REQUIRE(aux.ldes[0].height == lde_height, TS_ERR_INVALID,
               "aux data: LDE height is not the trace height << log_blowup");
}

std::vector<DeviceMatrix> TwoAdicFriPcs::quotient_chunks(const PcsData& trace_data,
                                                         const AirProgram& air,
                                                         const std::vector<uint32_t>& pis, Ef alpha,
                                                         const PcsData* preprocessed, const PcsData* aux) {
    TS_REQUIRE(trace_data.ldes.size() >= 1, TS_ERR_INVALID, "quotient: no trace matrix");
    TS_REQUIRE(trace_data.log_height >= fri_.log_blowup, TS_ERR_INVALID, "quotient: bad trace data");
    if (preprocessed) check_preprocessed_key(*preprocessed, air, trace_data.ldes[0].height);
    if (aux) check_third_matrix(*aux, air, trace_data.ldes[0].height);
    return quotient_chunks_slab(trace_data.ldes[0], trace_data.log_height - fri_.log_blowup, Slab{}, air,
                                pis, alpha, GENERATOR, preprocessed ? &preprocessed->ldes[0] : nullptr,
                                aux ? &aux->ldes[0] : nullptr);
}

std::vector<DeviceMatrix> TwoAdicFriPcs::quotient_chunks_slab(const ColMat& lde_slab, unsigned log_n,
                                                              const Slab& slab, const AirProgram& air,
                                                              const std::vector<uint32_t>& pis, Ef alpha,
                                                              uint32_t domain_shift, const ColMat* prep_lde,
                                                              const ColMat* aux_lde) {
    StageTimer t(&ctx_, "compute quotient polynomial");
    TS_REQUIRE((aux_lde != nullptr) == air.has_third(), TS_ERR_INVALID,
               "quotient: an AIR with preprocessed and aux columns needs both committed matrices, and only such an "
               "AIR takes two");
    TS_REQUIRE(!aux_lde || slab.rows == 0, TS_ERR_UNSUPPORTED, "quotient: aux columns beside preprocessed ones on a slab");
    TS_REQUIRE((prep_lde != nullptr) == (air.second_width() > 0), TS_ERR_INVALID,
               "quotient: an AIR with preprocessed columns needs their committed key, and only such an AIR takes one");
    TS_REQUIRE(!prep_lde || slab.rows == 0, TS_ERR_UNSUPPORTED, "quotient: preprocessed columns on a slab");
    TS_REQUIRE(lde_slab.width == air.width, TS_ERR_INVALID, "quotient: trace width != AIR width");
    TS_REQUIRE(pis.size() == air.n_public_slots(), TS_ERR_INVALID, "quotient: wrong number of public values");
    const unsigned lqd = air.log_quotient_degree;
    TS_REQUIRE(lqd <= fri_.log_blowup, TS_ERR_INVARIANT,
               "quotient domain larger than the committed LDE (log_quotient_degree > log_blowup)");
    const uint64_t n = 1ull << log_n, qn = n << lqd;
    const uint32_t qd = 1u << lqd;
    const uint64_t slab_rows = slab.rows ? slab.rows : lde_slab.height;
    const uint64_t row_begin = std::min<uint64_t>(slab.row0, qn);
    const uint64_t row_end = std::min<uint64_t>(slab.row0 + slab_rows, qn);
    TS_REQUIRE(row_begin % n == 0 && row_end % n == 0, TS_ERR_INVALID, "quotient: slab must hold whole cosets");

    std::vector<uint32_t> consts = air_consts_mont(air, pis.data(), pis.size());
    consts.resize((consts.size() + 3) & ~(size_t)3, 0);
    const size_t n_consts = consts.size();
    const uint32_t K = air.n_constraints;
    const std::vector<uint32_t> pw = alpha_powers_mont(alpha, K);
    consts.resize(n_consts + std::max<size_t>(4 * (size_t)K, 4), 0);
    for (uint32_t i = 0; i < K; i++) memcpy(&consts[n_consts + 4 * (size_t)(K - 1 - i)], &pw[4 * (size_t)i], 16);
    DevBuf<uint32_t> d_consts(&ctx_, consts.size());
    h2d(ctx_, d_consts.p, consts.data(), consts.size() * 4);

    std::vector<DeviceMatrix> chunks(qd);
    QuotOut qo;
    memset(&qo, 0, sizeof qo);
    for (uint32_t c = 0; c < qd; c++) {
        chunks[c].buf = DevBuf<uint32_t>(&ctx_, 4 * n);
        chunks[c].height = n;
        chunks[c].width = 4;
        chunks[c].layout = DeviceMatrix::COL_MAJOR_BITREV;
        qo.chunk[c] = chunks[c].buf.p;
    }
    if (row_begin < row_end) {
        ColMat lde = lde_slab;
        lde.d = lde_slab.d - slab.row0;
        launch_quotient(ctx_, air, lde, log_n, lqd, d_consts.p, d_consts.p + n_consts, qo, row_begin, row_end,
                        domain_shift, prep_lde, aux_lde);
    }
    return chunks;
}

DevBuf<Ef> TwoAdicFriPcs::open_reduce(const PcsData& trace_data, const PcsData& quotient_data, Ef zeta,
                                      Ef alpha, std::vector<Ef>& opened_values, const PcsData* preprocessed,
                                      const PcsData* aux) {
    TS_REQUIRE(trace_data.log_height == quotient_data.log_height, TS_ERR_INVALID,
               "open: trace and quotient LDE heights differ");
    return open_reduce_slab(trace_data, quotient_data, trace_data.log_height, Slab{}, zeta, alpha,
                            opened_values, preprocessed, aux);
}

DevBuf<Ef> TwoAdicFriPcs::open_reduce_slab(const PcsData& trace_data, const PcsData& quotient_data,
                                           unsigned log_N, const Slab& slab, Ef zeta, Ef alpha,
                                           std::vector<Ef>& opened_values, const PcsData* preprocessed,
                                           const PcsData* aux) {
    TS_REQUIRE(trace_data.ldes.size() == 1, TS_ERR_UNSUPPORTED, "open: one trace matrix expected");
    TS_REQUIRE(!aux || (preprocessed && slab.rows == 0 && aux->ldes.size() == 1 &&
                        aux->ldes[0].height == trace_data.ldes[0].height),
               TS_ERR_INVALID, "open: aux round shape");
    const ColMat* xm = aux ? &aux->ldes[0] : nullptr;
    const uint32_t aw = xm ? xm->width : 0;
    TS_REQUIRE(!preprocessed || (slab.rows == 0 && preprocessed->ldes.size() == 1 &&
                                 preprocessed->ldes[0].height == trace_data.ldes[0].height),
               TS_ERR_INVALID, "open: preprocessed round shape");
    const ColMat* pm = preprocessed ? &preprocessed->ldes[0] : nullptr;
    const uint32_t pw = pm ? pm->width : 0;
    const unsigned log_n = log_N - fri_.log_blowup;
    const uint64_t n = 1ull << log_n;
    const uint64_t N = slab.rows ? slab.rows : 1ull << log_N;
    TS_REQUIRE(N >= n && trace_data.ldes[0].height == N, TS_ERR_INVALID, "open: slab shape");
    const uint32_t coset_gen =
        mul(GENERATOR, pow_canon(two_adic_generator(log_N), bitrev32(slab.beta0, fri_.log_blowup)));
    const ColMat& tr = trace_data.ldes[0];
    const uint32_t w = tr.width;
    const uint32_t qd = (uint32_t)quotient_data.ldes.size();
    for (auto& m : quotient_data.ldes)
        TS_REQUIRE(m.width == 4, TS_ERR_INVALID, "open: quotient chunks must have width 4");
    ctx_.ensure_twiddles(std::max(1u, log_N));

    const Ef zeta_next = efc_mul_base(zeta, two_adic_generator(log_n));
    const Ef pts_mont[2] = {ef_to_mont(zeta), ef_to_mont(zeta_next)};

    std::vector<Ef> raw_all(2 * (size_t)pw + 2 * (size_t)aw + 2 * (size_t)w + 4 * (size_t)qd);
    Ef* const raw = raw_all.data() + 2 * (size_t)pw + 2 * (size_t)aw;
    DevBuf<Ef> weights(&ctx_, 2 * n);
    {
        StageTimer t(&ctx_, "compute opened values with Lagrange interpolation");
        launch_bary_weights(ctx_, log_n, pts_mont, 2, weights.p, coset_gen);
        Ef* const mail = reinterpret_cast<Ef*>(ctx_.mailbox(4 * raw_all.size()));
        struct { Ef* p; } sums{mail + 2 * (size_t)pw + 2 * (size_t)aw};
        BaryPending pend;
        if (pm) {
            pend.capacity = xm ? 4 : 3;
            launch_bary_dots(ctx_, *pm, log_n, weights.p, 2, mail, &pend);
        }
        if (xm) launch_bary_dots(ctx_, *xm, log_n, weights.p, 2, mail + 2 * (size_t)pw, &pend);
        launch_bary_dots(ctx_, tr, log_n, weights.p, 2, sums.p, &pend);
        ColMat all;
        if (qd > 1 && columns_as_one_matrix(quotient_data.ldes, quotient_data.ldes[0].height, 0, all) &&
            all.width == 4 * qd) {
            launch_bary_dots(ctx_, all, log_n, weights.p, 1, sums.p + 2 * w, &pend);
        } else {
            for (uint32_t c = 0; c < qd; c++)
                launch_bary_dots(ctx_, quotient_data.ldes[c], log_n, weights.p, 1, sums.p + 2 * w + 4 * c, &pend);
        }
        launch_bary_finish(ctx_, pend);
        ctx_.sync_point(mail, raw_all.size() * sizeof(Ef));
        memcpy(raw_all.data(), mail, raw_all.size() * sizeof(Ef));
    }
    const Ef scale[2] = {bary_scale(zeta, coset_gen, n), bary_scale(zeta_next, coset_gen, n)};
    opened_values.assign(raw_all.size(), ef_zero());
    for (uint32_t c = 0; c < pw; c++) {
        opened_values[c] = efc_mul(raw_all[2 * c], scale[0]);
        opened_values[pw + c] = efc_mul(raw_all[2 * c + 1], scale[1]);
    }
    for (uint32_t c = 0; c < aw; c++) {
        opened_values[2 * (size_t)pw + c] = efc_mul(raw_all[2 * (size_t)pw + 2 * c], scale[0]);
        opened_values[2 * (size_t)pw + aw + c] = efc_mul(raw_all[2 * (size_t)pw + 2 * c + 1], scale[1]);
    }
    Ef* const ov = opened_values.data() + 2 * (size_t)pw + 2 * (size_t)aw;
    for (uint32_t c = 0; c < w; c++) {
        ov[c] = efc_mul(raw[2 * c], scale[0]);
        ov[w + c] = efc_mul(raw[2 * c + 1], scale[1]);
    }
    for (uint32_t k = 0; k < 4 * qd; k++) ov[2 * w + k] = efc_mul(raw[2 * w + k], scale[0]);

    StageTimer t(&ctx_, "reduce rows");
    const uint32_t max_w = std::max(std::max(std::max(w, pw), aw), 4u);
    std::vector<uint32_t> apow = alpha_powers_mont(alpha, max_w);
    const Ef am = ef_to_mont(alpha);
    auto reduced_ys = [&](const Ef* ys, uint32_t width) {
        Ef acc = ef_zero();
        for (uint32_t i = 0; i < width; i++) {
            Ef ap;
            memcpy(ap.c, &apow[4 * (size_t)i], 16);
            acc = ef_add(acc, ef_mul(ys[i], ap));
        }
        return acc;
    };
    const bool low = slab.rows == 0 && !pm && reduce_low_wanted(w + 4 * qd);
    if (!low) weights.reset();
    DevBuf<Ef> ro(&ctx_, N);
    {
        TS_REQUIRE(qd <= (uint32_t)MAX_QUOTIENT_CHUNKS, TS_ERR_UNSUPPORTED, "open: more than 64 quotient chunks");
        FusedReduceArgs a;
        memset(&a, 0, sizeof a);
        a.z_mont[0] = pts_mont[0];
        a.z_mont[1] = pts_mont[1];
        uint64_t num_reduced = 0;
        Ef off_p[2] = {ef_zero(), ef_zero()}, kp[2] = {ef_zero(), ef_zero()};
        for (int p = 0; pm && p < 2; p++) {
            off_p[p] = ef_pow(am, num_reduced);
            kp[p] = ef_mul(reduced_ys(&opened_values[(size_t)p * pw], pw), off_p[p]);
            num_reduced += pw;
        }
        Ef off_a[2] = {ef_zero(), ef_zero()};
        for (int p = 0; xm && p < 2; p++) {
            off_a[p] = ef_pow(am, num_reduced);
            kp[p] = ef_add(kp[p], ef_mul(reduced_ys(&opened_values[2 * (size_t)pw + (size_t)p * aw], aw), off_a[p]));
            num_reduced += aw;
        }
        a.off_t[0] = ef_pow(am, num_reduced);
        a.k0 = ef_add(kp[0], ef_mul(reduced_ys(&ov[0], w), a.off_t[0]));
        num_reduced += w;
        a.off_t[1] = ef_pow(am, num_reduced);
        a.k1 = ef_add(kp[1], ef_mul(reduced_ys(&ov[w], w), a.off_t[1]));
        num_reduced += w;
        a.n_chunks = qd;
        a.chunk_stride = N;
        a.row0 = slab.row0;
        a.rows = N;
        std::vector<uint32_t> cw(16 * (size_t)qd);
        for (uint32_t c = 0; c < qd; c++) {
            TS_REQUIRE(quotient_data.ldes[c].col_stride == N, TS_ERR_INVALID, "open: chunk stride");
            a.chunk[c] = quotient_data.ldes[c].d;
            const Ef off_c = ef_pow(am, num_reduced);
            a.k0 = ef_add(a.k0, ef_mul(reduced_ys(&ov[2 * w + 4 * c], 4), off_c));
            for (int k = 0; k < 4; k++) {
                Ef ap;
                memcpy(ap.c, &apow[4 * (size_t)k], 16);
                const Ef wk = ef_mul(ap, off_c);
                memcpy(&cw[16 * (size_t)c + 4 * k], wk.c, 16);
            }
            num_reduced += 4;
        }
        const size_t n_apow = apow.size();
        apow.insert(apow.end(), cw.begin(), cw.end());
        DevBuf<uint32_t> d_apow(&ctx_, apow.size());
        h2d(ctx_, d_apow.p, apow.data(), apow.size() * 4);
        a.chunk_w = d_apow.p + n_apow;
        if (low) {
            DevBuf<uint32_t> ro_low(&ctx_, 4 * n), ro_cols(&ctx_, 4 * N);
            launch_reduce_low(ctx_, tr, log_n, d_apow.p, a, weights.p, ro_low.p);
            coset_lde(ctx_, ro_low.p, n, 4, log_n, fri_.log_blowup, 1, ro_cols.p, N, 0, 0, false, nullptr, 0, 0,
                      false);
            launch_ef_interleave(ctx_, ro_cols.p, N, N, ro.p);
        } else {
            launch_reduce_fused(ctx_, tr, log_N, d_apow.p, a, ro.p, pm, off_p, xm, off_a);
        }
    }
    return ro;
}

void TwoAdicFriPcs::open_batch(const PcsData& d, uint64_t index, std::vector<uint32_t>& rows,
                               std::vector<uint32_t>& path) {
    TS_REQUIRE(index < (1ull << d.log_height), TS_ERR_INVALID, "open_batch: index out of range");
    QueryGather qg(ctx_);
    const unsigned li = qg.add_indices({(uint32_t)index});
    const QueryGather::Slot o_rows = qg.add_rows(li, d.leaf_mats(), 0), o_path = qg.add_path(li, d.tree.p, d.log_height, 0);
    qg.run();
    rows.assign(qg.data(o_rows, 0), qg.data(o_rows, 0) + o_rows.words);
    path.assign(qg.data(o_path, 0), qg.data(o_path, 0) + o_path.words);
}

void TwoAdicFriPcs::fri_prove(std::vector<DevBuf<Ef>>& inputs, const std::vector<unsigned>& log_lens,
                              BfChallenger& challenger,
                              const std::vector<const PcsData*>& input_rounds,
                              std::vector<uint32_t>& pf, bool pass_through) {
    Context& ctx = ctx_;
    const FriConfig& fri = fri_;
    TS_REQUIRE(!inputs.empty() && inputs.size() == log_lens.size(), TS_ERR_INVALID, "FRI: no input");
    std::vector<const Ef*> in_ptr;
    for (auto& v : inputs) in_ptr.push_back(v.p);
    if (pass_through)
        TS_REQUIRE(input_rounds.empty() && log_lens.back() >= 1, TS_ERR_INVALID,
                   "FRI: pass-through input proof takes no committed batches");
    for (size_t k = 1; k < log_lens.size(); k++)
        TS_REQUIRE(log_lens[k] < log_lens[k - 1], TS_ERR_INVALID, "FRI: inputs must descend in height");
    const unsigned log_max_height = log_lens[0];
    TS_REQUIRE(log_lens.back() >= fri.log_blowup, TS_ERR_INVALID, "FRI: vector shorter than the blowup");
    for (const PcsData* d : input_rounds)
        TS_REQUIRE(d->log_height <= log_max_height, TS_ERR_INVALID,
                   "FRI: a committed batch is taller than every opened matrix");

    FriCommit st;
    Ef final_poly;
    {
        StageTimer t(&ctx, "FRI commit phase");
        fri_commit_begin(ctx, fri, log_max_height, challenger, st);
        fri_commit_rounds(ctx, fri, std::move(inputs[0]), 1ull << log_max_height, inputs, log_lens, 1, st);
        final_poly = fri_commit_finish(ctx, fri, challenger, st);
    }
    std::vector<FriRound>& rounds = st.rounds;
    const uint32_t R = (uint32_t)rounds.size();

    uint32_t pow_witness;
    {
        StageTimer t(&ctx, "grind for proof-of-work witness");
        pow_witness = fri_pow_witness(ctx, challenger, fri.proof_of_work_bits, st);
    }

    StageTimer tq(&ctx, "query phase");
    const uint32_t Q = fri.num_queries;
    std::vector<uint32_t> indices(Q);
    for (uint32_t q = 0; q < Q; q++) indices[q] = (uint32_t)challenger.sample_bits(log_max_height);

    const size_t n_in_rounds = input_rounds.size();
    QueryGather qg(ctx);
    const unsigned li = qg.add_indices(indices);
    std::vector<QueryGather::Slot> o_rows(n_in_rounds), o_path(n_in_rounds);
    for (size_t k = 0; k < n_in_rounds; k++) {
        const unsigned lh = input_rounds[k]->log_height;
        o_rows[k] = qg.add_rows(li, input_rounds[k]->leaf_mats(), log_max_height - lh);
        o_path[k] = qg.add_path(li, input_rounds[k]->tree.p, lh, log_max_height - lh);
    }
    std::vector<QueryGather::Opening> o_round(R);
    for (uint32_t r = 0; r < R; r++)
        o_round[r] = qg.add_round(li, rounds[r].vec, rounds[r].tree, rounds[r].log_leaves, r + 1);
    std::vector<QueryGather::Slot> o_pass(pass_through ? in_ptr.size() : 0);
    for (size_t k = 0; k < o_pass.size(); k++)
        o_pass[k] = qg.add_values(li, in_ptr[k], log_max_height - log_lens[k] + 1);
    qg.run();

    std::vector<ProofWriter::Batch> batches;
    for (const PcsData* d : input_rounds) batches.push_back({&d->ldes, d->log_height});
    std::vector<unsigned> round_depths;
    for (auto& r : rounds) round_depths.push_back(r.log_leaves);
    pf.reserve(pf.size() + 16 + 8 * (size_t)R +
               (size_t)Q * ProofWriter::words_per_query(batches, round_depths, o_pass.size()));
    ProofWriter pw(pf);
    pw.begin_rounds(R);
    for (uint32_t r = 0; r < R; r++) pw.commitment(rounds[r].root, 8);
    pw.begin_queries(Q);
    for (uint32_t q = 0; q < Q; q++) {
        pw.begin_input_proof((uint32_t)(pass_through ? in_ptr.size() : n_in_rounds));
        for (size_t k = 0; k < o_pass.size(); k++) {
            const uint32_t half = (indices[q] >> (log_max_height - log_lens[k])) & 1;
            pw.pass_through_value(log_lens[k], qg.data(o_pass[k], q) + 4 * half);
        }
        for (size_t k = 0; k < n_in_rounds; k++) {
            const unsigned lh = input_rounds[k]->log_height;
            pw.batch_opening(input_rounds[k]->ldes, qg.data(o_rows[k], q), lh, {{qg.data(o_path[k], q), lh}});
        }
        for (uint32_t r = 0; r < R; r++)
            pw.round_opening(qg.data(o_round[r].vals, q), rounds[r].log_leaves,
                             {{qg.data(o_round[r].path, q), rounds[r].log_leaves}});
    }
    pw.finish(final_poly, pow_witness);
}

std::vector<uint32_t> TwoAdicFriPcs::open(const std::vector<OpenRound>& rounds, BfChallenger& challenger,
                                          std::vector<Ef>& opened_values) {
    TS_REQUIRE(!rounds.empty(), TS_ERR_INVALID, "open: no rounds");
    const Ef alpha = challenger.sample();
    const Ef am = ef_to_mont(alpha);
    uint32_t max_w = 1;
    unsigned log_global_max = 0;
    for (auto& r : rounds) {
        TS_REQUIRE(r.data && r.points.size() == r.data->ldes.size(), TS_ERR_INVALID,
                   "open: one point list per committed matrix");
        for (auto& m : r.data->ldes) max_w = std::max(max_w, m.width);
        log_global_max = std::max(log_global_max, r.data->log_height);
    }
    ctx_.ensure_twiddles(std::max(1u, log_global_max));
    const std::vector<uint32_t> apow = alpha_powers_mont(alpha, max_w);
    DevBuf<uint32_t> d_apow(&ctx_, apow.size());
    h2d(ctx_, d_apow.p, apow.data(), apow.size() * 4);

    opened_values.clear();
    DevBuf<Ef> ro[32];
    uint64_t num_reduced[32] = {0};
    for (auto& r : rounds) {
        for (size_t mi = 0; mi < r.data->ldes.size(); mi++) {
            const ColMat& m = r.data->ldes[mi];
            const unsigned log_h = log2_strict(m.height);
            TS_REQUIRE(log_h >= fri_.log_blowup, TS_ERR_INVALID, "open: matrix shorter than the blowup");
            const unsigned log_n = log_h - fri_.log_blowup;
            const uint64_t n = 1ull << log_n;
            const uint32_t w = m.width;
            const auto& pts = r.points[mi];
            for (size_t p0 = 0; p0 < pts.size(); p0 += 2) {
                const uint32_t np = (uint32_t)std::min<size_t>(2, pts.size() - p0);
                Ef pts_mont[2] = {ef_to_mont(pts[p0]), ef_to_mont(pts[p0 + np - 1])};
                std::vector<Ef> raw((size_t)w * np);
                {
                    StageTimer t(&ctx_, "compute opened values with Lagrange interpolation");
                    DevBuf<Ef> weights(&ctx_, (size_t)np * n);
                    launch_bary_weights(ctx_, log_n, pts_mont, np, weights.p);
                    DevBuf<Ef> sums(&ctx_, raw.size());
                    launch_bary_dots(ctx_, m, log_n, weights.p, np, sums.p);
                    d2h_sync(ctx_, raw.data(), sums.p, raw.size() * sizeof(Ef));
                }
                StageTimer t(&ctx_, "reduce rows");
                ReduceArgs a;
                memset(&a, 0, sizeof a);
                a.n_points = np;
                for (uint32_t p = 0; p < np; p++) {
                    const Ef scale = bary_scale(pts[p0 + p], GENERATOR, n);
                    Ef rys = ef_zero();
                    for (uint32_t c = 0; c < w; c++) {
                        const Ef y = efc_mul(raw[(size_t)c * np + p], scale);
                        opened_values.push_back(y);
                        Ef ap;
                        memcpy(ap.c, &apow[4 * (size_t)c], 16);
                        rys = ef_add(rys, ef_mul(y, ap));
                    }
                    a.z_mont[p] = pts_mont[p];
                    a.off_mont[p] = ef_pow(am, num_reduced[log_h]);
                    a.rys[p] = rys;
                    num_reduced[log_h] += w;
                }
                if (!ro[log_h].p) {
                    ro[log_h] = DevBuf<Ef>(&ctx_, m.height);
                    a.accumulate = 0;
                } else {
                    a.accumulate = 1;
                }
                launch_reduce(ctx_, m, log_h, d_apow.p, a, ro[log_h].p);
            }
        }
    }
    std::vector<DevBuf<Ef>> inputs;
    std::vector<unsigned> log_lens;
    for (int lh = 31; lh >= 0; lh--)
        if (ro[lh].p) {
            inputs.push_back(std::move(ro[lh]));
            log_lens.push_back((unsigned)lh);
        }
    TS_REQUIRE(!inputs.empty(), TS_ERR_INVALID, "open: nothing to open");
    TS_REQUIRE(log_lens[0] == log_global_max, TS_ERR_UNSUPPORTED,
               "open: the tallest committed matrix must be opened at one point at least");
    std::vector<const PcsData*> datas;
    for (auto& r : rounds) datas.push_back(r.data);
    std::vector<uint32_t> pf;
    fri_prove(inputs, log_lens, challenger, datas, pf);
    return pf;
}

std::vector<uint32_t> prove(TwoAdicFriPcs& pcs, const AirProgram& air, BfChallenger& challenger,
                            DeviceMatrix trace, const std::vector<uint32_t>& public_values,
                            const PcsData* preprocessed, uint32_t proof_version) {
    const Statement st = check_statement(pcs.fri(), air, trace.width, trace.height, public_values.size());
    TS_REQUIRE((preprocessed != nullptr) == (air.preprocessed_width > 0), TS_ERR_INVALID,
               "prove: an AIR with preprocessed columns needs their committed key, and only such an AIR takes one");
    if (preprocessed) {
        check_preprocessed_key(*preprocessed, air, 1ull << st.log_N);
        challenger.observe_commitment(preprocessed->root);
    }
    pcs.ctx().ensure_twiddles(std::max(1u, st.log_N));

    std::vector<DeviceMatrix> tv;
    tv.push_back(std::move(trace));
    std::unique_ptr<PcsData> trace_data = pcs.commit(tv, {1u});
    challenger.observe_commitment(trace_data->root);
    const Ef alpha = challenger.sample();

    std::vector<DeviceMatrix> chunks = pcs.quotient_chunks(*trace_data, air, public_values, alpha, preprocessed);
    std::unique_ptr<PcsData> quotient_data =
        pcs.commit(chunks, chunk_domain_shifts(GENERATOR, st.log_degree, st.lqd));
    challenger.observe_commitment(quotient_data->root);
    const Ef zeta = challenger.sample();

    const Ef batch_alpha = challenger.sample();
    std::vector<Ef> opened;
    std::vector<DevBuf<Ef>> inputs;
    inputs.push_back(pcs.open_reduce(*trace_data, *quotient_data, zeta, batch_alpha, opened, preprocessed));

    std::vector<uint32_t> pf;
    pf.reserve(64 + opened.size() * 4);
    ProofWriter pw(pf);
    pw.header(proof_version, st.log_degree, st.w, st.qd, air.preprocessed_width);
    pw.commitment(trace_data->root, 8);
    pw.commitment(quotient_data->root, 8);
    pw.opened_values(opened);
    std::vector<const PcsData*> rounds{trace_data.get(), quotient_data.get()};
    if (preprocessed) rounds.insert(rounds.begin(), preprocessed);
    pcs.fri_prove(inputs, {st.log_N}, challenger, rounds, pf);
    return pf;
}

static std::vector<uint32_t> prove_challenge_phase(TwoAdicFriPcs& pcs, const AirProgram& air, BfChallenger& challenger,
                                                   DeviceMatrix trace, const std::vector<uint32_t>& public_values,
                                                   const AuxSource& aux_source, const PcsData* preprocessed,
                                                   uint32_t proof_version) {
    const Statement st = check_statement(pcs.fri(), air, trace.width, trace.height, public_values.size());
    TS_REQUIRE(proof_version == 5 || air.preprocessed_width == 0, TS_ERR_UNSUPPORTED,
               "prove_aux: preprocessed columns together with aux columns need a third matrix in the kernels");
    TS_REQUIRE((preprocessed != nullptr) == (air.preprocessed_width > 0), TS_ERR_INVALID,
               "prove: an AIR with preprocessed columns needs their committed key, and only such an AIR takes one");
    const uint32_t aw = air.aux_width;
    TS_REQUIRE((aux_source != nullptr) == (aw > 0), TS_ERR_INVALID,
               "prove_aux: an AIR with aux columns needs an aux source, and only such an AIR takes one");
    TS_REQUIRE(aw > 0 || air.n_exposed == 0, TS_ERR_INVALID, "prove_aux: exposed words without aux columns");
    TS_REQUIRE(!aw || trace.layout == DeviceMatrix::ROW_MAJOR, TS_ERR_INVALID,
               "prove_aux: the trace must be row-major (it is handed to the aux source after its commit)");
    if (preprocessed) {
        check_preprocessed_key(*preprocessed, air, 1ull << st.log_N);
        challenger.observe_commitment(preprocessed->root);
    }
    pcs.ctx().ensure_twiddles(std::max(1u, st.log_N));
    const uint64_t n = trace.height;

    std::vector<DeviceMatrix> tv;
    tv.push_back(std::move(trace));
    std::unique_ptr<PcsData> trace_data = pcs.commit(tv, {1u}, true, aw > 0);
    challenger.observe_commitment(trace_data->root);
    std::vector<uint32_t> pis = public_values;
    for (uint32_t k = 0; k < air.n_challenges; k++) {
        const Ef c = challenger.sample();
        pis.insert(pis.end(), c.c, c.c + 4);
    }
    std::unique_ptr<PcsData> aux_data;
    std::vector<uint32_t> exposed(air.n_exposed, 0);
    if (aw) {
        DeviceMatrix aux = aux_source(tv[0], pis.data() + public_values.size(), exposed.data());
        tv[0].buf.reset();
        TS_REQUIRE(aux.buf.p && aux.buf.ctx == &pcs.ctx(), TS_ERR_INVALID,
                   "prove_aux: the aux matrix is consumed or was made on another context");
        TS_REQUIRE(aux.height == n && aux.width == aw, TS_ERR_INVALID,
                   "prove_aux: the aux matrix must have the trace's height and the AIR's aux width");
        for (uint32_t e : exposed) TS_REQUIRE(e < P, TS_ERR_INVALID, "prove_aux: non-canonical exposed word");
        std::vector<DeviceMatrix> av;
        av.push_back(std::move(aux));
        aux_data = pcs.commit(av, {1u});
        challenger.observe_commitment(aux_data->root);
        for (uint32_t e : exposed) challenger.observe(e);
    }
    pis.insert(pis.end(), exposed.begin(), exposed.end());
    const Ef alpha = challenger.sample();

    const PcsData* second = preprocessed ? preprocessed : aux_data.get();
    const PcsData* third = preprocessed ? aux_data.get() : nullptr;
    std::vector<DeviceMatrix> chunks = pcs.quotient_chunks(*trace_data, air, pis, alpha, second, third);
    std::unique_ptr<PcsData> quotient_data =
        pcs.commit(chunks, chunk_domain_shifts(GENERATOR, st.log_degree, st.lqd));
    challenger.observe_commitment(quotient_data->root);
    const Ef zeta = challenger.sample();

    const Ef batch_alpha = challenger.sample();
    std::vector<Ef> opened;
    std::vector<DevBuf<Ef>> inputs;
    inputs.push_back(pcs.open_reduce(*trace_data, *quotient_data, zeta, batch_alpha, opened, second, third));

    std::vector<uint32_t> pf;
    pf.reserve(64 + exposed.size() + opened.size() * 4);
    ProofWriter pw(pf);
    pw.header(proof_version, st.log_degree, st.w, st.qd, aw);
    const uint32_t more[3] = {air.n_challenges, air.n_exposed, air.preprocessed_width};
    pw.words(more, proof_version == 5 ? 3 : 2);
    pw.commitment(trace_data->root, 8);
    if (aw) {
        pw.commitment(aux_data->root, 8);
        pw.words(exposed.data(), exposed.size());
    }
    pw.commitment(quotient_data->root, 8);
    pw.opened_values(opened);
    std::vector<const PcsData*> rounds{trace_data.get(), quotient_data.get()};
    if (aw) rounds.insert(rounds.begin(), aux_data.get());
    if (preprocessed) rounds.insert(rounds.begin(), preprocessed);
    pcs.fri_prove(inputs, {st.log_N}, challenger, rounds, pf);
    return pf;
}

std::vector<uint32_t> prove_aux(TwoAdicFriPcs& pcs, const AirProgram& air, BfChallenger& challenger,
                                DeviceMatrix trace, const std::vector<uint32_t>& public_values,
                                const AuxSource& aux_source) {
    return prove_challenge_phase(pcs, air, challenger, std::move(trace), public_values, aux_source, nullptr, 4);
}

std::vector<uint32_t> prove_pre_aux(TwoAdicFriPcs& pcs, const AirProgram& air, BfChallenger& challenger,
                                    DeviceMatrix trace, const std::vector<uint32_t>& public_values,
                                    const PcsData* preprocessed, const AuxSource& aux_source) {
    return prove_challenge_phase(pcs, air, challenger, std::move(trace), public_values, aux_source, preprocessed, 5);
}

}
```

tap-stark_amd/csrc/prover_common.cpp:

```cpp
#include <stdlib.h>
#include <string.h>

#include <optional>

#include "prover_internal.hpp"

namespace ts {

void h2d(Context& ctx, void* dst, const void* src, size_t bytes) {
    if (!bytes) return;
    const void* from = bytes <= (1u << 20) ? ctx.stage(src, bytes) : src;
    TS_HIP(hipMemcpyAsync(dst, from, bytes, hipMemcpyHostToDevice, ctx.stream));
}
void d2h_sync(Context& ctx, void* dst, const void* src, size_t bytes) {
    if (bytes) TS_HIP(hipMemcpyAsync(dst, src, bytes, hipMemcpyDeviceToHost, ctx.stream));
    ctx.sync();
}

unsigned log2_strict(uint64_t n) {
    unsigned k = 0;
    while ((1ull << k) < n) k++;
    TS_REQUIRE((1ull << k) == n, TS_ERR_INVALID, "height must be a power of two");
    return k;
}

Ef efc_mul(Ef a, Ef b) { return ef_mul(a, ef_to_mont(b)); }
Ef efc_mul_base(Ef a, uint32_t b) { return ef_mul_base(a, to_mont(b)); }
Ef efc_pow(Ef a, uint64_t e) { return ef_from_mont(ef_pow(ef_to_mont(a), e)); }

std::vector<const uint32_t*> column_pointers(const std::vector<ColMat>& ldes, uint64_t height) {
    std::vector<const uint32_t*> cols;
    for (auto& cm : ldes)
        if (!height || cm.height == height)
            for (uint32_t c = 0; c < cm.width; c++) cols.push_back(cm.d + (uint64_t)c * cm.col_stride);
    return cols;
}

bool columns_as_one_matrix(const std::vector<ColMat>& ldes, uint64_t height, uint32_t max_width, ColMat& one) {
    const ColMat* first = nullptr;
    uint32_t wsum = 0;
    for (auto& cm : ldes)
        if (cm.height == height) {
            if (!first) first = &cm;
            if (cm.col_stride != first->col_stride || cm.d != first->d + (uint64_t)wsum * first->col_stride)
                return false;
            wsum += cm.width;
        }
    if (!wsum || (max_width && wsum > max_width)) return false;
    one = *first;
    one.width = wsum;
    return true;
}

LeafMats PcsData::leaf_mats() const {
    LeafMats lm;
    memset(&lm, 0, sizeof lm);
    lm.n_mats = (uint32_t)ldes.size();
    for (size_t i = 0; i < ldes.size(); i++) {
        lm.d[i] = ldes[i].d;
        lm.col_stride[i] = ldes[i].col_stride;
        lm.width[i] = ldes[i].width;
        lm.row_shift[i] = (uint8_t)(log_height - log2_strict(ldes[i].height));
        lm.total_width += ldes[i].width;
    }
    lm.cols = col_table_uploaded ? col_table.p : nullptr;
    return lm;
}

LeafMats PcsData::leaf_mats_with_table(Context& ctx) {
    if (!col_table_uploaded) {
        const std::vector<const uint32_t*> cols = column_pointers(ldes);
        col_table = DevBuf<const uint32_t*>(&ctx, cols.size());
        h2d(ctx, col_table.p, cols.data(), cols.size() * sizeof(const uint32_t*));
        col_table_uploaded = true;
    }
    return leaf_mats();
}

void lde_stage(Context& ctx, const FriConfig& fri, std::vector<DeviceMatrix>& evals,
               const std::vector<uint32_t>& domain_shifts, uint32_t beta0, uint32_t n_beta, bool allow_pair,
               PcsData& data, bool keep_row_major) {
    TS_REQUIRE(!evals.empty() && evals.size() <= (size_t)MAX_BATCH_MATS, TS_ERR_INVALID,
               "commit: between 1 and MAX_BATCH_MATS (64) matrices per batch");
    TS_REQUIRE(evals.size() == domain_shifts.size(), TS_ERR_INVALID, "commit: one domain per matrix");
    uint64_t max_n = 0;
    bool same_height = true;
    size_t total_w = 0;
    for (size_t i = 0; i < evals.size(); i++) {
        const DeviceMatrix& m = evals[i];
        TS_REQUIRE(m.width >= 1 && m.buf.p, TS_ERR_INVALID, "commit: empty matrix");
        TS_REQUIRE(domain_shifts[i] != 0 && domain_shifts[i] < P, TS_ERR_INVALID, "bad domain shift");
        log2_strict(m.height);
        max_n = std::max(max_n, m.height);
        same_height = same_height && m.height == evals[0].height;
        total_w += m.width;
    }
    TS_REQUIRE(same_height || !n_beta, TS_ERR_INVALID, "sharded commit: matrices of one height expected");
    const unsigned log_N = log2_strict(max_n) + fri.log_blowup;
    TS_REQUIRE(log_N <= 27, TS_ERR_INVALID, "commit: LDE larger than the two-adic subgroup");
    ctx.ensure_twiddles(std::max(1u, log_N));
    auto lde_rows = [&](uint64_t n) { return n_beta ? (uint64_t)n_beta * n : n << fri.log_blowup; };
    data.log_height = log2_strict(lde_rows(max_n));
    auto push_lde = [&](uint32_t* d, uint64_t rows, uint32_t width) {
        ColMat cm;
        cm.d = d;
        cm.height = rows;
        cm.width = width;
        cm.col_stride = rows;
        data.ldes.push_back(cm);
    };

    StageTimer t(&ctx, "coset_lde");
    const bool batched = same_height && evals.size() > 1;
    DevBuf<uint32_t> batch;
    if (batched) batch = DevBuf<uint32_t>(&ctx, total_w * lde_rows(evals[0].height));
    size_t batch_col = 0;
    static const bool pair_knob = [] { const char* e = getenv("TS_LDE_PAIR"); return !e || atoi(e) != 0; }();
    if (allow_pair && pair_knob && batched && evals.size() == 2 && evals[0].width == evals[1].width &&
        evals[0].layout == DeviceMatrix::COL_MAJOR_BITREV && evals[1].layout == DeviceMatrix::COL_MAJOR_BITREV) {
        const uint64_t n = evals[0].height, rows = lde_rows(n);
        const uint32_t w = evals[0].width;
        coset_lde(ctx, evals[0].buf.p, n, 2 * w, log2_strict(n), fri.log_blowup,
                  mul(GENERATOR, inv_canon(domain_shifts[0])), batch.p, rows, beta0, n_beta, false, evals[1].buf.p,
                  mul(GENERATOR, inv_canon(domain_shifts[1])), w);
        for (size_t i = 0; i < 2; i++) {
            push_lde(batch.p + i * (size_t)w * rows, rows, w);
            evals[i].buf.reset();
        }
        data.lde_storage.push_back(std::move(batch));
        return;
    }
    for (size_t i = 0; i < evals.size(); i++) {
        DeviceMatrix& m = evals[i];
        const uint64_t n = m.height, rows = lde_rows(n);
        const unsigned log_n = log2_strict(n);
        DevBuf<uint32_t> colmajor;
        uint32_t* ev = m.buf.p;
        bool r16 = false;
        if (m.layout == DeviceMatrix::ROW_MAJOR) {
            std::optional<StageTimer> tt;
            if (n_beta) tt.emplace(&ctx, "lde: transpose (every column on every rank)");
            colmajor = DevBuf<uint32_t>(&ctx, (size_t)m.width * n);
            r16 = launch_transpose_bitrev_r16(ctx, m.buf.p, colmajor.p, log_n, m.width, n);
            if (!r16) launch_transpose_bitrev(ctx, m.buf.p, colmajor.p, log_n, m.width, n);
            ev = colmajor.p;
        }
        DevBuf<uint32_t> own;
        uint32_t* lde;
        if (batched) {
            lde = batch.p + batch_col * rows;
            batch_col += m.width;
        } else {
            own = DevBuf<uint32_t>(&ctx, (size_t)m.width * rows);
            lde = own.p;
        }
        coset_lde(ctx, ev, n, m.width, log_n, fri.log_blowup, mul(GENERATOR, inv_canon(domain_shifts[i])), lde,
                  rows, beta0, n_beta, r16);
        push_lde(lde, rows, m.width);
        if (!batched) data.lde_storage.push_back(std::move(own));
        if (!(keep_row_major && m.layout == DeviceMatrix::ROW_MAJOR)) m.buf.reset();
    }
    if (batched) data.lde_storage.push_back(std::move(batch));
}

bool reduce_low_wanted(uint32_t opened_columns) {
    if (const char* e = getenv("TS_REDUCE_LOW"); e && *e) return atoi(e) != 0;
    return opened_columns >= REDUCE_LOW_MIN_WIDTH;
}

Statement check_statement(const FriConfig& fri, const AirProgram& air, uint32_t trace_width, uint64_t degree,
                          size_t n_public_values) {
    TS_REQUIRE(trace_width == air.width, TS_ERR_INVALID, "prove: trace width != AIR width");
    TS_REQUIRE(n_public_values == air.n_public, TS_ERR_INVALID, "prove: wrong number of public values");
    Statement s;
    s.log_degree = log2_strict(degree);
    s.lqd = air.log_quotient_degree;
    s.qd = 1u << s.lqd;
    s.log_N = s.log_degree + fri.log_blowup;
    s.w = air.width;
    TS_REQUIRE(s.lqd <= fri.log_blowup, TS_ERR_INVARIANT,
               "quotient domain larger than the committed LDE (log_quotient_degree > log_blowup)");
    return s;
}

std::vector<uint32_t> air_consts_mont(const AirProgram& air, const uint32_t* pis, size_t n) {
    TS_REQUIRE(n == air.n_public_slots(), TS_ERR_INVALID, "wrong number of public values");
    std::vector<uint32_t> consts(std::max<size_t>(air.const_canonical.size(), 1), 0);
    for (size_t k = 0; k < air.const_canonical.size(); k++) {
        const uint32_t v = air.const_public_idx[k] != ~0u ? pis[air.const_public_idx[k]] : air.const_canonical[k];
        TS_REQUIRE(v < P, TS_ERR_INVALID, "non-canonical public value");
        consts[k] = to_mont(v);
    }
    return consts;
}

std::vector<uint32_t> alpha_powers_mont(Ef alpha, size_t count) {
    std::vector<uint32_t> pw(4 * count);
    const Ef am = ef_to_mont(alpha);
    Ef cur = ef_one_mont();
    for (size_t i = 0; i < count; i++) {
        memcpy(&pw[4 * i], cur.c, 16);
        cur = ef_mul(cur, am);
    }
    return pw;
}

Ef bary_scale(Ef point, uint32_t coset_gen, uint64_t n) {
    Ef un = efc_pow(efc_mul_base(point, inv_canon(coset_gen)), n);
    un.c[0] = sub(un.c[0], 1);
    return efc_mul_base(un, inv_canon((uint32_t)(n % P)));
}

std::vector<uint32_t> chunk_domain_shifts(uint32_t base_shift, unsigned log_degree, unsigned lqd) {
    std::vector<uint32_t> shifts(1u << lqd);
    const uint32_t gq = two_adic_generator(log_degree + lqd);
    for (uint32_t c = 0; c < shifts.size(); c++) shifts[c] = mul(base_shift, pow_canon(gq, c));
    return shifts;
}

size_t ProofWriter::words_per_query(const std::vector<Batch>& batches, const std::vector<unsigned>& round_depths,
                                    size_t n_pass_through) {
    size_t n = 1 + 5 * n_pass_through;
    for (auto& b : batches) {
        n += 1 + b.mats->size() + 1 + 8 * (size_t)b.depth;
        for (auto& m : *b.mats) n += m.width;
    }
    for (unsigned d : round_depths) n += 8 + 1 + 8 * (size_t)d;
    return n;
}

void ProofWriter::header(uint32_t version, unsigned log_degree, uint32_t width, uint32_t qd, uint32_t extra) {
    out_.push_back(TSPF_MAGIC);
    out_.push_back(version);
    out_.push_back(log_degree);
    out_.push_back(width);
    out_.push_back(qd);
    if (version >= 2) out_.push_back(extra);
}

void ProofWriter::opened_values(const std::vector<Ef>& values) {
    for (auto& e : values) words(e.c, 4);
}

void ProofWriter::path(std::initializer_list<Path> parts) {
    for (auto& part : parts) {
        if (!swap_) words(part.digests, 8 * part.depth);
        else for (size_t k = 0; k < 8 * part.depth; k++) out_.push_back(__builtin_bswap32(part.digests[k]));
    }
}

void ProofWriter::pass_through_value(unsigned log_height, const uint32_t value[4]) {
    out_.push_back(log_height);
    words(value, 4);
}

void ProofWriter::batch_opening(const std::vector<ColMat>& mats, const uint32_t* row, unsigned depth,
                                std::initializer_list<Path> parts) {
    out_.push_back((uint32_t)mats.size());
    for (auto& m : mats) {
        out_.push_back(m.width);
        words(row, m.width);
        row += m.width;
    }
    out_.push_back(depth);
    path(parts);
}

void ProofWriter::round_opening(const uint32_t values[8], unsigned depth, std::initializer_list<Path> parts) {
    words(values, 8);
    out_.push_back(depth);
    path(parts);
}

void ProofWriter::finish(Ef final_poly, uint32_t pow_witness) {
    words(final_poly.c, 4);
    out_.push_back(pow_witness);
}

unsigned QueryGather::add_indices(const std::vector<uint32_t>& indices) {
    lists_.emplace_back();
    lists_.back().indices = indices;
    return (unsigned)lists_.size() - 1;
}

QueryGather::Slot QueryGather::take(const List& l, size_t words_per_query) {
    const Slot s{words_, words_per_query};
    words_ += l.indices.size() * words_per_query;
    return s;
}

QueryGather::Slot QueryGather::add_rows(unsigned list, const LeafMats& mats, unsigned shift) {
    List& l = lists_.at(list);
    const Slot s = take(l, mats.total_width);
    RowGatherJob jb{};
    jb.mats = mats;
    jb.shift = shift;
    jb.out = s.at;
    l.rows.push_back(jb);
    l.max_row_width = std::max(l.max_row_width, mats.total_width);
    return s;
}

QueryGather::Opening QueryGather::add_desc(unsigned list, const Ef* vec, const uint32_t* tree, unsigned log_leaves,
                                           unsigned shift) {
    List& l = lists_.at(list);
    FriGatherDesc d{};
    d.vec = reinterpret_cast<const uint32_t*>(vec);
    d.tree = tree;
    d.log_leaves = log_leaves;
    d.shift = shift;
    Opening o;
    if (vec) d.out_vals = (o.vals = take(l, 8)).at;
    if (tree) d.out_path = (o.path = take(l, 8 * (size_t)log_leaves)).at;
    l.descs.push_back(d);
    l.max_log_leaves = std::max(l.max_log_leaves, d.log_leaves);
    return o;
}
QueryGather::Slot QueryGather::add_path(unsigned list, const uint32_t* tree, unsigned log_leaves, unsigned shift) {
    return add_desc(list, nullptr, tree, log_leaves, shift).path;
}
QueryGather::Opening QueryGather::add_round(unsigned list, const Ef* vec, const uint32_t* tree, unsigned log_leaves,
                                            unsigned shift) {
    return add_desc(list, vec, tree, log_leaves, shift);
}
QueryGather::Slot QueryGather::add_values(unsigned list, const Ef* vec, unsigned shift) {
    return add_desc(list, vec, nullptr, 0, shift).vals;
}

void QueryGather::run() {
    static_assert(sizeof(RowGatherJob) % 8 == 0 && sizeof(FriGatherDesc) % 8 == 0, "tables stay 8-byte aligned");
    size_t b_rows = 0, b_descs = 0, b_idx = 0;
    for (auto& l : lists_) {
        b_rows += l.rows.size() * sizeof(RowGatherJob);
        b_descs += l.descs.size() * sizeof(FriGatherDesc);
        b_idx += l.indices.size() * 4;
    }
    if (!b_idx) return;
    std::vector<unsigned char> up(b_rows + b_descs + b_idx);
    auto put = [](unsigned char*& at, const void* src, size_t bytes) {
        if (bytes) memcpy(at, src, bytes);
        at += bytes;
    };
    unsigned char *rows = up.data(), *descs = rows + b_rows, *idx = descs + b_descs;
    for (auto& l : lists_) {
        put(rows, l.rows.data(), l.rows.size() * sizeof(RowGatherJob));
        put(descs, l.descs.data(), l.descs.size() * sizeof(FriGatherDesc));
        put(idx, l.indices.data(), l.indices.size() * 4);
    }
    DevBuf<unsigned char> d_up(&ctx_, up.size());
    h2d(ctx_, d_up.p, up.data(), up.size());
    DevBuf<uint32_t> d_out(&ctx_, std::max<size_t>(words_, 1));
    rows = d_up.p, descs = rows + b_rows, idx = descs + b_descs;
    for (auto& l : lists_) {
        launch_gather_queries(ctx_, reinterpret_cast<const RowGatherJob*>(rows), (uint32_t)l.rows.size(),
                              l.max_row_width, reinterpret_cast<const FriGatherDesc*>(descs), (uint32_t)l.descs.size(),
                              l.max_log_leaves, reinterpret_cast<const uint32_t*>(idx), (uint32_t)l.indices.size(),
                              d_out.p);
        rows += l.rows.size() * sizeof(RowGatherJob);
        descs += l.descs.size() * sizeof(FriGatherDesc);
        idx += l.indices.size() * 4;
    }
    out_.resize(words_);
    d2h_sync(ctx_, out_.data(), d_out.p, words_ * 4);
}

double bench_stage(Context& c, int stage, unsigned log_n, uint32_t width, unsigned log_blowup, uint32_t reps) {
    TS_REQUIRE(stage >= 0 && stage <= 4 && width >= 1 && width <= 256 && reps >= 1 && log_n >= 1 &&
                   log_n + log_blowup <= 27,
               TS_ERR_INVALID, "bench_stage: stage 0 .. 4, width 1..256, log_n + log_blowup <= 27");
    struct MaskGuard {
        Context& c;
        ~MaskGuard() { c.lde_pass_mask = 7; }
    } guard_mask{c};
    if (stage >= 2) {
        TS_REQUIRE(ntt_plan(log_n).two_pass, TS_ERR_INVALID, "bench_stage: single LDE passes exist for log_n > 12 only");
        c.lde_pass_mask = 1u << (stage - 2);
    }
    const bool is_lde = stage != 1;
    const uint64_t n = 1ull << log_n, N = n << log_blowup;
    c.ensure_twiddles(log_n + log_blowup);
    DevBuf<uint32_t> lde(&c, (size_t)width * N), in(&c, is_lde ? (size_t)width * n : 1);
    TS_HIP(hipMemsetAsync(lde.p, 0x11, (size_t)width * N * 4, c.stream));
    if (is_lde) TS_HIP(hipMemsetAsync(in.p, 0x11, (size_t)width * n * 4, c.stream));
    DevBuf<uint32_t> tree(&c, stage == 1 ? merkle_total_digests(log_n + log_blowup) * 8 : 1);
    std::vector<const uint32_t*> cols(width);
    for (uint32_t k = 0; k < width; k++) cols[k] = lde.p + (uint64_t)k * N;
    DevBuf<const uint32_t*> d_cols(&c, width);
    TS_HIP(hipMemcpyAsync(d_cols.p, cols.data(), width * sizeof(const uint32_t*), hipMemcpyHostToDevice, c.stream));
    c.sync();
    LeafMats lm;
    memset(&lm, 0, sizeof lm);
    lm.n_mats = 1;
    lm.d[0] = lde.p;
    lm.col_stride[0] = N;
    lm.width[0] = width;
    lm.total_width = width;
    lm.cols = d_cols.p;
    auto once = [&] {
        if (is_lde) coset_lde(c, in.p, n, width, log_n, log_blowup, GENERATOR, lde.p, N);
        else launch_commit_tree(c, lm, log_n + log_blowup, tree.p);
    };
    once();
    hipEvent_t e0, e1;
    TS_HIP(hipEventCreate(&e0));
    TS_HIP(hipEventCreate(&e1));
    TS_HIP(hipEventRecord(e0, c.stream));
    for (uint32_t r = 0; r < reps; r++) once();
    TS_HIP(hipEventRecord(e1, c.stream));
    c.sync();
    float ms = 0;
    TS_HIP(hipEventElapsedTime(&ms, e0, e1));
    (void)hipEventDestroy(e0);
    (void)hipEventDestroy(e1);
    return (double)ms / reps;
}

}
```

tap-stark_amd/csrc/prover_internal.hpp:

```cpp
#pragma once
#include <functional>
#include <initializer_list>

#include "host.hpp"

namespace ts {

struct FriRound {
    const Ef* vec = nullptr;
    const uint32_t* tree = nullptr;
    unsigned log_leaves = 0;
    uint32_t root[8];
};

struct FriCommit {
    DevBuf<Ef> cur;
    const Ef* deferred = nullptr;
    uint64_t len = 0;
    using TopStep = std::function<void(const uint32_t* d_subroot, size_t round)>;
    void round(Context& ctx, bool defer_next, const TopStep& top = nullptr, uint64_t h_global = 0, uint64_t row0 = 0);

    std::vector<FriRound> rounds;
    std::vector<DevBuf<Ef>> keep_vecs;
    std::vector<DevBuf<uint32_t>> keep_trees;
    DevBuf<uint32_t> d_block;
    struct { uint32_t* p = nullptr; } d_chal, d_roots;
    struct { Ef* p = nullptr; } d_final;
    DevBuf<Ef> d_betas;
    uint32_t R_total = 0;
    uint64_t final_len = 0;
    uint32_t pow_hint = 0xffffffffu;
    DevChallenger* dch() { return reinterpret_cast<DevChallenger*>(d_chal.p); }
};
constexpr size_t FRI_POW_WORD = 40;

void fri_commit_begin(Context& ctx, const FriConfig& fri, unsigned log_max_height,
                      const BfChallenger& challenger, FriCommit& st);
void fri_commit_rounds(Context& ctx, const FriConfig& fri, DevBuf<Ef> folded, uint64_t len,
                       std::vector<DevBuf<Ef>>& inputs, const std::vector<unsigned>& log_lens,
                       size_t next_in, FriCommit& st);
Ef fri_commit_finish(Context& ctx, const FriConfig& fri, BfChallenger& challenger, FriCommit& st);
uint32_t fri_pow_witness(Context& ctx, BfChallenger& challenger, unsigned bits, const FriCommit& st);

void lde_stage(Context& ctx, const FriConfig& fri, std::vector<DeviceMatrix>& evals,
               const std::vector<uint32_t>& domain_shifts, uint32_t beta0, uint32_t n_beta, bool allow_pair,
               PcsData& data, bool keep_row_major = false);

constexpr uint32_t REDUCE_LOW_MIN_WIDTH = 72;
bool reduce_low_wanted(uint32_t opened_columns);

struct Statement {
    unsigned log_degree, lqd;
    uint32_t qd;
    unsigned log_N;
    uint32_t w;
};
Statement check_statement(const FriConfig& fri, const AirProgram& air, uint32_t trace_width, uint64_t degree,
                          size_t n_public_values);

std::vector<uint32_t> air_consts_mont(const AirProgram& air, const uint32_t* pis, size_t n);
std::vector<uint32_t> alpha_powers_mont(Ef alpha, size_t count);
Ef bary_scale(Ef point, uint32_t coset_gen, uint64_t n);
std::vector<uint32_t> chunk_domain_shifts(uint32_t base_shift, unsigned log_degree, unsigned lqd);

constexpr uint32_t TSPF_MAGIC = 0x46505354u;
class ProofWriter {
public:
    struct Path { const uint32_t* digests; size_t depth; };
    struct Batch { const std::vector<ColMat>* mats; unsigned depth; };
    explicit ProofWriter(std::vector<uint32_t>& out, bool swap_path_bytes = false)
        : out_(out), swap_(swap_path_bytes) {}
    static size_t words_per_query(const std::vector<Batch>& batches, const std::vector<unsigned>& round_depths,
                                  size_t n_pass_through = 0);

    void words(const uint32_t* p, size_t n) { out_.insert(out_.end(), p, p + n); }
    void header(uint32_t version, unsigned log_degree, uint32_t width, uint32_t qd, uint32_t extra);
    void commitment(const uint32_t* roots, size_t n_words) { words(roots, n_words); }
    void opened_values(const std::vector<Ef>& values);
    void begin_rounds(uint32_t n_rounds) { out_.push_back(n_rounds); }
    void begin_queries(uint32_t n_queries) { out_.push_back(n_queries); }
    void begin_input_proof(uint32_t n) { out_.push_back(n); }
    void pass_through_value(unsigned log_height, const uint32_t value[4]);
    void batch_opening(const std::vector<ColMat>& mats, const uint32_t* row, unsigned depth,
                       std::initializer_list<Path> path);
    void round_opening(const uint32_t values[8], unsigned depth, std::initializer_list<Path> path);
    void finish(Ef final_poly, uint32_t pow_witness);

private:
    void path(std::initializer_list<Path> parts);
    std::vector<uint32_t>& out_;
    bool swap_;
};

class QueryGather {
public:
    struct Slot { size_t at = 0, words = 0; };
    struct Opening { Slot vals, path; };
    explicit QueryGather(Context& ctx) : ctx_(ctx) {}
    unsigned add_indices(const std::vector<uint32_t>& indices);
    Slot add_rows(unsigned list, const LeafMats& mats, unsigned shift);
    Slot add_path(unsigned list, const uint32_t* tree, unsigned log_leaves, unsigned shift);
    Opening add_round(unsigned list, const Ef* vec, const uint32_t* tree, unsigned log_leaves, unsigned shift);
    Slot add_values(unsigned list, const Ef* vec, unsigned shift);
    void run();
    const uint32_t* data(Slot s, size_t query) const { return out_.data() + s.at + query * s.words; }

private:
    struct List {
        std::vector<uint32_t> indices;
        std::vector<RowGatherJob> rows;
        std::vector<FriGatherDesc> descs;
        uint32_t max_row_width = 0, max_log_leaves = 0;
    };
    Slot take(const List& l, size_t words_per_query);
    Opening add_desc(unsigned list, const Ef* vec, const uint32_t* tree, unsigned log_leaves, unsigned shift);
    Context& ctx_;
    std::vector<List> lists_;
    std::vector<uint32_t> out_;
    size_t words_ = 0;
};

void h2d(Context& ctx, void* dst, const void* src, size_t bytes);
void d2h_sync(Context& ctx, void* dst, const void* src, size_t bytes);
Ef efc_mul(Ef a, Ef b);
Ef efc_mul_base(Ef a, uint32_t b);
Ef efc_pow(Ef a, uint64_t e);

}
```

Baseline: 25.96 billion.

## Fuse opening reduction into barycentric dot pass and defer opened-value readback

The barycentric dot kernel gains a template mode that also emits per-row alpha-weighted sums for each column tile. A small finish kernel then builds the FRI input from these sums and GPU-computed constants, so the separate trace re-read of the reduce-low path is no longer needed. Opened values stay in a held pinned mailbox slot and are written into the proof only after the FRI commit phase, which removes a host sync between opening and FRI. This adds per-row output buffers, an extra code path enabled by default (controlled by TS_OPEN_ONE_PASS), and mailbox hold bookkeeping that could collide with other mailbox users.

```diff
diff --git a/tap-stark_amd/csrc/context.cpp b/tap-stark_amd/csrc/context.cpp
--- a/tap-stark_amd/csrc/context.cpp
+++ b/tap-stark_amd/csrc/context.cpp
@@ -173,7 +173,7 @@
 }
 
 uint32_t* Context::mailbox(size_t words) {
-    constexpr size_t WORDS = 16384;
+    constexpr size_t WORDS = MAILBOX_WORDS;
     if (words > WORDS / 4) {
         if (words > h_mailbox_big_words) {
             sync();
@@ -188,9 +188,20 @@
     if (!h_mailbox) TS_HIP(hipHostMalloc((void**)&h_mailbox, WORDS * 4, hipHostMallocDefault));
     const size_t need = (words + 15) & ~(size_t)15;
     if (mailbox_off + need > WORDS) mailbox_off = 0;
+    if (mailbox_off < mailbox_hold_end && mailbox_off + need > mailbox_hold_begin) {
+        mailbox_off = mailbox_hold_end;
+        if (mailbox_off + need > WORDS) mailbox_off = 0;
+    }
     uint32_t* p = h_mailbox + mailbox_off;
     mailbox_off += need;
     return p;
+}
+
+void Context::mailbox_hold(const uint32_t* slot, size_t words) {
+    TS_REQUIRE(mailbox_hold_begin == mailbox_hold_end, TS_ERR_INVARIANT, "mailbox: a slot is held already");
+    if (!h_mailbox || slot < h_mailbox || slot >= h_mailbox + MAILBOX_WORDS) return;
+    mailbox_hold_begin = (size_t)(slot - h_mailbox);
+    mailbox_hold_end = mailbox_hold_begin + ((words + 15) & ~(size_t)15);
 }
 
 void* Context::pinned(size_t bytes) {
diff --git a/tap-stark_amd/csrc/context.hpp b/tap-stark_amd/csrc/context.hpp
--- a/tap-stark_amd/csrc/context.hpp
+++ b/tap-stark_amd/csrc/context.hpp
@@ -87,11 +87,15 @@
 
     unsigned lde_pass_mask = 7;
 
+    static constexpr size_t MAILBOX_WORDS = 16384;
     uint32_t* h_mailbox = nullptr;
     size_t mailbox_off = 0;
     uint32_t* h_mailbox_big = nullptr;
     size_t h_mailbox_big_words = 0;
     uint32_t* mailbox(size_t words);
+    size_t mailbox_hold_begin = 0, mailbox_hold_end = 0;
+    void mailbox_hold(const uint32_t* slot, size_t words);
+    void mailbox_release() { mailbox_hold_begin = mailbox_hold_end = 0; }
 
     void* h_pinned = nullptr;
     size_t h_pinned_bytes = 0;
diff --git a/tap-stark_amd/csrc/host.hpp b/tap-stark_amd/csrc/host.hpp
--- a/tap-stark_amd/csrc/host.hpp
+++ b/tap-stark_amd/csrc/host.hpp
@@ -1,5 +1,6 @@
 #pragma once
 #include <stdint.h>
+#include <string.h>
 
 #include <algorithm>
 #include <functional>
@@ -77,6 +78,26 @@
 
 void mmcs_commit(Context& ctx, PcsData& data);
 
+struct PendingOpened {
+    Context* ctx = nullptr;
+    const Ef* mail = nullptr;
+    uint32_t w = 0, qd = 0;
+    Ef scale[2];
+    size_t at = 0;
+    PendingOpened() = default;
+    PendingOpened(const PendingOpened&) = delete;
+    PendingOpened& operator=(const PendingOpened&) = delete;
+    ~PendingOpened() { release(); }
+    bool active() const { return mail != nullptr; }
+    size_t count() const { return 2 * (size_t)w + 4 * (size_t)qd; }
+    std::vector<Ef> values();
+    void fill(std::vector<uint32_t>& proof) {
+        const std::vector<Ef> v = values();
+        if (!v.empty()) memcpy(&proof[at], v.data(), v.size() * sizeof(Ef));
+    }
+    void release();
+};
+
 class TwoAdicFriPcs {
 public:
     TwoAdicFriPcs(Context& ctx, FriConfig fri) : ctx_(ctx), fri_(fri) {}
@@ -93,7 +114,7 @@
 
     DevBuf<Ef> open_reduce(const PcsData& trace_data, const PcsData& quotient_data, Ef zeta,
                            Ef batch_alpha, std::vector<Ef>& opened_values, const PcsData* preprocessed = nullptr,
-                           const PcsData* aux = nullptr);
+                           const PcsData* aux = nullptr, PendingOpened* later = nullptr);
 
     struct Slab {
         uint64_t row0 = 0, rows = 0;
@@ -106,7 +127,8 @@
                                                    const ColMat* prep_lde = nullptr, const ColMat* aux_lde = nullptr);
     DevBuf<Ef> open_reduce_slab(const PcsData& trace_data, const PcsData& quotient_data, unsigned log_N,
                                 const Slab& slab, Ef zeta, Ef batch_alpha, std::vector<Ef>& opened_values,
-                                const PcsData* preprocessed = nullptr, const PcsData* aux = nullptr);
+                                const PcsData* preprocessed = nullptr, const PcsData* aux = nullptr,
+                                PendingOpened* later = nullptr);
 
     struct OpenRound {
         const PcsData* data = nullptr;
@@ -117,12 +139,14 @@
 
     void fri_prove(std::vector<DevBuf<Ef>>& inputs, const std::vector<unsigned>& log_lens,
                    BfChallenger& challenger, const std::vector<const PcsData*>& input_rounds,
-                   std::vector<uint32_t>& pf, bool pass_through = false);
+                   std::vector<uint32_t>& pf, bool pass_through = false, PendingOpened* opened_later = nullptr);
 
     void open_batch(const PcsData& d, uint64_t index, std::vector<uint32_t>& rows,
                     std::vector<uint32_t>& path);
 
 private:
+    DevBuf<Ef> open_reduce_one_pass(const ColMat& tr, const ColMat& chunks, unsigned log_N, Ef zeta, Ef alpha,
+                                    std::vector<Ef>& opened_values, PendingOpened* later);
     Context& ctx_;
     FriConfig fri_;
 };
diff --git a/tap-stark_amd/csrc/kernels.hpp b/tap-stark_amd/csrc/kernels.hpp
--- a/tap-stark_amd/csrc/kernels.hpp
+++ b/tap-stark_amd/csrc/kernels.hpp
@@ -113,8 +113,14 @@
     uint32_t n_blocks[4] = {0, 0, 0, 0}, n_words[4] = {0, 0, 0, 0};
     uint32_t n = 0, capacity = 2;
 };
+struct BaryRowSums {
+    const uint32_t* col_w;
+    Ef* out;
+};
+inline uint32_t bary_tile_columns(uint32_t width) { return width <= 8 ? 8 : 64; }
+inline uint32_t bary_column_tiles(uint32_t width) { return (width + bary_tile_columns(width) - 1) / bary_tile_columns(width); }
 void launch_bary_dots(Context& ctx, const ColMat& m, unsigned log_n, const Ef* weights,
-                      uint32_t n_points, Ef* out, BaryPending* pending = nullptr);
+                      uint32_t n_points, Ef* out, BaryPending* pending = nullptr, const BaryRowSums* rows = nullptr);
 void launch_bary_finish(Context& ctx, BaryPending& pending);
 struct ReduceArgs {
     Ef z_mont[2];
@@ -141,6 +147,11 @@
                          const ColMat* aux = nullptr, const Ef* aux_off_mont = nullptr);
 void launch_reduce_low(Context& ctx, const ColMat& trace, unsigned log_n, const uint32_t* d_alpha_pows_mont,
                        const FusedReduceArgs& args, const Ef* weights, uint32_t* out);
+void launch_open_consts(Context& ctx, const Ef* raw, uint32_t w, uint32_t n_chunk_cols, const uint32_t* col_w,
+                        const uint32_t* chunk_w, Ef m0_mont, Ef m1_mont, Ef s0_mont, Ef* mail, Ef* k);
+void launch_reduce_low_finish(Context& ctx, unsigned log_n, const Ef* row_t, uint32_t tiles_t, const Ef* row_c,
+                              uint32_t tiles_c, Ef off_t0_mont, Ef off_t1_mont, const Ef* k, const Ef* weights,
+                              uint32_t* out);
 void launch_ef_interleave(Context& ctx, const uint32_t* cols, uint64_t col_stride, uint64_t rows, Ef* out);
 
 void launch_fri_fold(Context& ctx, const Ef* in, uint64_t h, Ef beta_canonical, Ef* out,
diff --git a/tap-stark_amd/csrc/open.hip b/tap-stark_amd/csrc/open.hip
--- a/tap-stark_amd/csrc/open.hip
+++ b/tap-stark_amd/csrc/open.hip
@@ -60,10 +60,11 @@
     TS_HIP(hipGetLastError());
 }
 
-template <int NP, int COLS>
+template <int NP, int COLS, bool ROWS>
 __global__ void __launch_bounds__(256)
 k_bary_dots(const uint32_t* __restrict__ m, uint64_t col_stride, uint32_t width, unsigned log_n,
-            const Ef* __restrict__ weights, uint32_t* __restrict__ partial, uint32_t rows_per_block) {
+            const Ef* __restrict__ weights, uint32_t* __restrict__ partial, uint32_t rows_per_block,
+            const uint32_t* __restrict__ col_w, uint32_t* __restrict__ row_out) {
     constexpr int RS = 64 / COLS;
     constexpr int TR = 16 * 4 * RS;
     constexpr int PER_THREAD = COLS * TR / 256;
@@ -77,6 +78,10 @@
     const uint32_t sub = wv * RS + rs;
     const uint64_t row_begin = (uint64_t)blockIdx.x * rows_per_block;
     const uint64_t row_end = row_begin + rows_per_block < n ? row_begin + rows_per_block : n;
+    constexpr int KR = TR >= 256 ? TR / 256 : 1;
+    constexpr int KC = TR >= 256 ? 1 : 256 / TR;
+    const uint32_t et = threadIdx.x % TR, ec = threadIdx.x / TR;
+    const uint32_t* __restrict__ mp = m + ((uint64_t)(c0 + ec) * col_stride + et);
     uint64_t acc[NP * 4];
 #pragma unroll
     for (int j = 0; j < NP * 4; j++) acc[j] = 0;
@@ -84,10 +89,8 @@
         uint32_t v[PER_THREAD];
 #pragma unroll
         for (int k = 0; k < PER_THREAD; k++) {
-            const uint32_t e = threadIdx.x + (uint32_t)k * 256;
-            const uint32_t c = c0 + e / TR;
-            const uint64_t t = row0 + e % TR;
-            v[k] = (c < width && t < row_end) ? m[(uint64_t)c * col_stride + t] : 0u;
+            const uint32_t dc = (uint32_t)(k / KR) * KC, dt = (uint32_t)(k % KR) * 256;
+            v[k] = (c0 + ec + dc < width && row0 + et + dt < row_end) ? mp[(uint64_t)dc * col_stride + (row0 + dt)] : 0u;
         }
         for (uint32_t e = threadIdx.x; e < (uint32_t)(TR * NP); e += 256) {
             const uint32_t p = e / TR, tt = e % TR;
@@ -101,9 +104,8 @@
         }
 #pragma unroll
         for (int k = 0; k < PER_THREAD; k++) {
-            const uint32_t e = threadIdx.x + (uint32_t)k * 256;
-            const uint32_t t = e % TR;
-            tile[(t & 15) * 257 + (t >> 4) * COLS + e / TR] = v[k];
+            const uint32_t t = et + (uint32_t)(k % KR) * 256;
+            tile[(t & 15) * 257 + (t >> 4) * COLS + ec + (uint32_t)(k / KR) * KC] = v[k];
         }
         __syncthreads();
 #pragma unroll
@@ -117,8 +119,55 @@
                 for (int j = 0; j < NP * 4; j++) acc[j] = lazy_fix(acc[j]);
             }
         }
+        if constexpr (ROWS && COLS == 64) {
+            const uint32_t cg = 16u * (uint32_t)__builtin_amdgcn_readfirstlane((int)wv);
+            const uint32_t* __restrict__ ap = col_w + 4 * (size_t)(c0 + cg);
+            const uint32_t* trow = tile + (lane & 15) * 257 + (lane >> 4) * COLS + cg;
+            uint64_t s[4] = {0, 0, 0, 0};
+#pragma unroll 4
+            for (int i = 0; i < 16; i++) {
+                const uint32_t x = trow[i];
+#pragma unroll
+                for (int j = 0; j < 4; j++) s[j] = lazy_mac(s[j], x, ap[4 * i + j]);
+                if (i & 1) {
+#pragma unroll
+                    for (int j = 0; j < 4; j++) s[j] = lazy_fix(s[j]);
+                }
+            }
+#pragma unroll
+            for (int j = 0; j < 4; j++) red[wv][lane][j] = lazy_finish(s[j]);
+        }
+        if constexpr (ROWS && COLS == 8) {
+            const uint32_t* __restrict__ ap = col_w + 4 * (size_t)c0;
+#pragma unroll
+            for (int h = 0; h < TR / 256; h++) {
+                const uint32_t tt = threadIdx.x + 256u * h;
+                const uint32_t* trow = tile + (tt & 15) * 257 + (tt >> 4) * COLS;
+                uint64_t s[4] = {0, 0, 0, 0};
+#pragma unroll
+                for (int i = 0; i < COLS; i++) {
+                    const uint32_t x = trow[i];
+#pragma unroll
+                    for (int j = 0; j < 4; j++) s[j] = lazy_mac(s[j], x, ap[4 * i + j]);
+                    if (i & 1) {
+#pragma unroll
+                        for (int j = 0; j < 4; j++) s[j] = lazy_fix(s[j]);
+                    }
+                }
+                if (row0 + tt < row_end)
+                    *reinterpret_cast<uint4*>(row_out + 4 * ((uint64_t)blockIdx.y * n + row0 + tt)) =
+                        make_uint4(lazy_finish(s[0]), lazy_finish(s[1]), lazy_finish(s[2]), lazy_finish(s[3]));
+            }
+        }
         __syncthreads();
-    }
+        if constexpr (ROWS && COLS == 64) {
+            const uint32_t r = threadIdx.x >> 2, j = threadIdx.x & 3;
+            if (row0 + r < row_end)
+                row_out[4 * ((uint64_t)blockIdx.y * n + row0 + r) + j] =
+                    add(add(red[0][r][j], red[1][r][j]), add(red[2][r][j], red[3][r][j]));
+        }
+    }
+    if constexpr (ROWS && COLS == 64) __syncthreads();
 #pragma unroll
     for (int j = 0; j < NP * 4; j++) red[sub][cl][j] = lazy_finish(acc[j]);
     __syncthreads();
@@ -206,7 +255,7 @@
 }
 
 void launch_bary_dots(Context& ctx, const ColMat& m, unsigned log_n, const Ef* weights,
-                      uint32_t n_points, Ef* out, BaryPending* pending) {
+                      uint32_t n_points, Ef* out, BaryPending* pending, const BaryRowSums* rows) {
     const uint64_t n = 1ull << log_n;
     const bool narrow = m.width <= 8;
     const uint32_t tr = narrow ? 512 : 64;
@@ -217,23 +266,26 @@
     const uint32_t n_words = m.width * n_points * 4;
     DevBuf<uint32_t> partial(&ctx, (size_t)n_blocks * n_words);
     const uint32_t* md = m.d;
+    const dim3 grid(n_blocks, bary_column_tiles(m.width));
+    const uint32_t* const cw = rows ? rows->col_w : nullptr;
+    uint32_t* const ro = rows ? reinterpret_cast<uint32_t*>(rows->out) : nullptr;
+#define TS_BARY_DOTS(NP, COLS, ROWS)                                                                          \
+    TS_LAUNCH(ctx, (k_bary_dots<NP, COLS, ROWS>), grid, dim3(256), 0, md, m.col_stride, m.width, log_n, weights, \
+              partial.p, rows_per_block, cw, ro)
     if (narrow) {
-        dim3 grid(n_blocks, (m.width + 7) / 8);
-        if (n_points == 2)
-            TS_LAUNCH(ctx, (k_bary_dots<2, 8>), grid, dim3(256), 0, md, m.col_stride, m.width, log_n,
-                      weights, partial.p, rows_per_block);
-        else
-            TS_LAUNCH(ctx, (k_bary_dots<1, 8>), grid, dim3(256), 0, md, m.col_stride, m.width, log_n,
-                      weights, partial.p, rows_per_block);
+        if (n_points == 2) {
+            if (rows) TS_BARY_DOTS(2, 8, true); else TS_BARY_DOTS(2, 8, false);
+        } else {
+            if (rows) TS_BARY_DOTS(1, 8, true); else TS_BARY_DOTS(1, 8, false);
+        }
     } else {
-        dim3 grid(n_blocks, (m.width + 63) / 64);
-        if (n_points == 2)
-            TS_LAUNCH(ctx, (k_bary_dots<2, 64>), grid, dim3(256), 0, md, m.col_stride, m.width, log_n,
-                      weights, partial.p, rows_per_block);
-        else
-            TS_LAUNCH(ctx, (k_bary_dots<1, 64>), grid, dim3(256), 0, md, m.col_stride, m.width, log_n,
-                      weights, partial.p, rows_per_block);
-    }
+        if (n_points == 2) {
+            if (rows) TS_BARY_DOTS(2, 64, true); else TS_BARY_DOTS(2, 64, false);
+        } else {
+            if (rows) TS_BARY_DOTS(1, 64, true); else TS_BARY_DOTS(1, 64, false);
+        }
+    }
+#undef TS_BARY_DOTS
     TS_HIP(hipGetLastError());
     BaryPending own;
     BaryPending& pend = pending ? *pending : own;
@@ -548,6 +600,17 @@
     return Ef{{lazy_finish(acc[0]), lazy_finish(acc[1]), lazy_finish(acc[2]), lazy_finish(acc[3])}};
 }
 
+__device__ __forceinline__ Ef reduce_low_row(Ef St, Ef D, Ef off_t0, Ef off_t1, Ef k0, Ef k1, unsigned log_n,
+                                             const uint32_t* __restrict__ Winv, uint32_t gen_inv_mont,
+                                             const Ef* __restrict__ weights, uint64_t t) {
+    const uint64_t n = 1ull << log_n;
+    const uint32_t nxi = neg(mont_mul(gen_inv_mont, root_bitrev(Winv, log_n, t)));
+    const Ef inv_d0 = ef_mul_base(weights[t], nxi), inv_d1 = ef_mul_base(weights[n + t], nxi);
+    const Ef g0 = ef_sub(ef_add(ef_mul(St, off_t0), D), k0);
+    const Ef g1 = ef_sub(ef_mul(St, off_t1), k1);
+    return ef_add(ef_mul(g0, inv_d0), ef_mul(g1, inv_d1));
+}
+
 __global__ void __launch_bounds__(256)
 k_reduce_low(const uint32_t* __restrict__ trace, uint64_t trace_stride, uint32_t width, unsigned log_n,
              const uint32_t* __restrict__ Winv, uint32_t gen_inv_mont, const uint32_t* __restrict__ alpha_pows,
@@ -557,11 +620,7 @@
     if (t >= n) return;
     const Ef St = row_dot_alpha(trace, trace_stride, width, t, alpha_pows);
     const Ef D = chunk_dot(a, t);
-    const uint32_t nxi = neg(mont_mul(gen_inv_mont, root_bitrev(Winv, log_n, t)));
-    const Ef inv_d0 = ef_mul_base(weights[t], nxi), inv_d1 = ef_mul_base(weights[n + t], nxi);
-    const Ef g0 = ef_sub(ef_add(ef_mul(St, a.off_t[0]), D), a.k0);
-    const Ef g1 = ef_sub(ef_mul(St, a.off_t[1]), a.k1);
-    const Ef r = ef_add(ef_mul(g0, inv_d0), ef_mul(g1, inv_d1));
+    const Ef r = reduce_low_row(St, D, a.off_t[0], a.off_t[1], a.k0, a.k1, log_n, Winv, gen_inv_mont, weights, t);
 #pragma unroll
     for (int k = 0; k < 4; k++) out[(uint64_t)k * n + t] = r.c[k];
 }
@@ -580,6 +639,81 @@
 }
 
 __global__ void __launch_bounds__(256)
+k_open_consts(const Ef* __restrict__ raw, uint32_t w, uint32_t n_chunk_cols, const uint32_t* __restrict__ col_w,
+              const uint32_t* __restrict__ chunk_w, Ef m0, Ef m1, Ef s0, Ef* __restrict__ mail, Ef* __restrict__ k) {
+    __shared__ uint32_t red[4][12];
+    Ef a0 = ef_zero(), a1 = ef_zero(), c = ef_zero();
+    for (uint32_t i = threadIdx.x; i < w; i += 256) {
+        const Ef ap = *reinterpret_cast<const Ef*>(col_w + 4 * (size_t)i);
+        const Ef r0 = raw[2 * (size_t)i], r1 = raw[2 * (size_t)i + 1];
+        mail[2 * (size_t)i] = r0;
+        mail[2 * (size_t)i + 1] = r1;
+        a0 = ef_add(a0, ef_mul(r0, ap));
+        a1 = ef_add(a1, ef_mul(r1, ap));
+    }
+    for (uint32_t i = threadIdx.x; i < n_chunk_cols; i += 256) {
+        const Ef r = raw[2 * (size_t)w + i];
+        mail[2 * (size_t)w + i] = r;
+        c = ef_add(c, ef_mul(r, *reinterpret_cast<const Ef*>(chunk_w + 4 * (size_t)i)));
+    }
+    uint32_t v[12] = {a0.c[0], a0.c[1], a0.c[2], a0.c[3], a1.c[0], a1.c[1], a1.c[2], a1.c[3],
+                      c.c[0],  c.c[1],  c.c[2],  c.c[3]};
+    const uint32_t lane = threadIdx.x & 63, wv = threadIdx.x >> 6;
+#pragma unroll
+    for (int j = 0; j < 12; j++) {
+#pragma unroll
+        for (int off = 32; off >= 1; off >>= 1) v[j] = add(v[j], __shfl_down(v[j], off, 64));
+        if (lane == 0) red[wv][j] = v[j];
+    }
+    __syncthreads();
+    if (threadIdx.x == 0) {
+        Ef t[3];
+#pragma unroll
+        for (int e = 0; e < 3; e++)
+#pragma unroll
+            for (int j = 0; j < 4; j++)
+                t[e].c[j] = add(add(red[0][4 * e + j], red[1][4 * e + j]), add(red[2][4 * e + j], red[3][4 * e + j]));
+        k[0] = ef_add(ef_mul(t[0], m0), ef_mul(t[2], s0));
+        k[1] = ef_mul(t[1], m1);
+    }
+}
+
+void launch_open_consts(Context& ctx, const Ef* raw, uint32_t w, uint32_t n_chunk_cols, const uint32_t* col_w,
+                        const uint32_t* chunk_w, Ef m0_mont, Ef m1_mont, Ef s0_mont, Ef* mail, Ef* k) {
+    TS_LAUNCH(ctx, k_open_consts, dim3(1), dim3(256), 0, raw, w, n_chunk_cols, col_w, chunk_w, m0_mont, m1_mont,
+              s0_mont, mail, k);
+    TS_HIP(hipGetLastError());
+}
+
+__global__ void __launch_bounds__(256)
+k_reduce_low_finish(unsigned log_n, const uint32_t* __restrict__ Winv, uint32_t gen_inv_mont,
+                    const Ef* __restrict__ row_t, uint32_t tiles_t, const Ef* __restrict__ row_c, uint32_t tiles_c,
+                    Ef off_t0, Ef off_t1, const Ef* __restrict__ k, const Ef* __restrict__ weights,
+                    uint32_t* __restrict__ out) {
+    const uint64_t n = 1ull << log_n;
+    const uint64_t t = (uint64_t)blockIdx.x * blockDim.x + threadIdx.x;
+    if (t >= n) return;
+    Ef St = row_t[t], D = row_c[t];
+    for (uint32_t i = 1; i < tiles_t; i++) St = ef_add(St, row_t[(uint64_t)i * n + t]);
+    for (uint32_t i = 1; i < tiles_c; i++) D = ef_add(D, row_c[(uint64_t)i * n + t]);
+    const Ef r = reduce_low_row(St, D, off_t0, off_t1, k[0], k[1], log_n, Winv, gen_inv_mont, weights, t);
+#pragma unroll
+    for (int j = 0; j < 4; j++) out[(uint64_t)j * n + t] = r.c[j];
+}
+
+void launch_reduce_low_finish(Context& ctx, unsigned log_n, const Ef* row_t, uint32_t tiles_t, const Ef* row_c,
+                              uint32_t tiles_c, Ef off_t0_mont, Ef off_t1_mont, const Ef* k, const Ef* weights,
+                              uint32_t* out) {
+    TS_REQUIRE(tiles_t >= 1 && tiles_c >= 1, TS_ERR_INVALID, "reduce_low_finish: no row sums");
+    const uint64_t n = 1ull << log_n;
+    ctx.ensure_twiddles(log_n == 0 ? 1 : log_n);
+    TS_LAUNCH_NAMED(ctx, "k_reduce_low", k_reduce_low_finish, dim3((unsigned)((n + 255) / 256)), dim3(256), 0, log_n,
+                    (const uint32_t*)ctx.d_twiddle_inv, to_mont(inv_canon(GENERATOR)), row_t, tiles_t, row_c, tiles_c,
+                    off_t0_mont, off_t1_mont, k, weights, out);
+    TS_HIP(hipGetLastError());
+}
+
+__global__ void __launch_bounds__(256)
 k_ef_interleave(const uint32_t* __restrict__ cols, uint64_t col_stride, uint64_t rows, Ef* __restrict__ out) {
     const uint64_t X = (uint64_t)blockIdx.x * blockDim.x + threadIdx.x;
     if (X >= rows) return;
diff --git a/tap-stark_amd/csrc/prover.cpp b/tap-stark_amd/csrc/prover.cpp
--- a/tap-stark_amd/csrc/prover.cpp
+++ b/tap-stark_amd/csrc/prover.cpp
@@ -167,17 +167,17 @@
 
 DevBuf<Ef> TwoAdicFriPcs::open_reduce(const PcsData& trace_data, const PcsData& quotient_data, Ef zeta,
                                       Ef alpha, std::vector<Ef>& opened_values, const PcsData* preprocessed,
-                                      const PcsData* aux) {
+                                      const PcsData* aux, PendingOpened* later) {
     TS_REQUIRE(trace_data.log_height == quotient_data.log_height, TS_ERR_INVALID,
                "open: trace and quotient LDE heights differ");
     return open_reduce_slab(trace_data, quotient_data, trace_data.log_height, Slab{}, zeta, alpha,
-                            opened_values, preprocessed, aux);
+                            opened_values, preprocessed, aux, later);
 }
 
 DevBuf<Ef> TwoAdicFriPcs::open_reduce_slab(const PcsData& trace_data, const PcsData& quotient_data,
                                            unsigned log_N, const Slab& slab, Ef zeta, Ef alpha,
                                            std::vector<Ef>& opened_values, const PcsData* preprocessed,
-                                           const PcsData* aux) {
+                                           const PcsData* aux, PendingOpened* later) {
     TS_REQUIRE(trace_data.ldes.size() == 1, TS_ERR_UNSUPPORTED, "open: one trace matrix expected");
     TS_REQUIRE(!aux || (preprocessed && slab.rows == 0 && aux->ldes.size() == 1 &&
                         aux->ldes[0].height == trace_data.ldes[0].height),
@@ -202,6 +202,17 @@
         TS_REQUIRE(m.width == 4, TS_ERR_INVALID, "open: quotient chunks must have width 4");
     ctx_.ensure_twiddles(std::max(1u, log_N));
 
+    const bool low = slab.rows == 0 && !pm && reduce_low_wanted(w + 4 * qd);
+    if (low && open_one_pass_wanted(ctx_)) {
+        ColMat all;
+        if (qd == 1) all = quotient_data.ldes[0];
+        if (qd == 1 || (columns_as_one_matrix(quotient_data.ldes, quotient_data.ldes[0].height, 0, all) &&
+                        all.width == 4 * qd)) {
+            TS_REQUIRE(all.col_stride == N, TS_ERR_INVALID, "open: chunk stride");
+            return open_reduce_one_pass(tr, all, log_N, zeta, alpha, opened_values, later);
+        }
+    }
+
     const Ef zeta_next = efc_mul_base(zeta, two_adic_generator(log_n));
     const Ef pts_mont[2] = {ef_to_mont(zeta), ef_to_mont(zeta_next)};
 
@@ -243,11 +254,7 @@
         opened_values[2 * (size_t)pw + aw + c] = efc_mul(raw_all[2 * (size_t)pw + 2 * c + 1], scale[1]);
     }
     Ef* const ov = opened_values.data() + 2 * (size_t)pw + 2 * (size_t)aw;
-    for (uint32_t c = 0; c < w; c++) {
-        ov[c] = efc_mul(raw[2 * c], scale[0]);
-        ov[w + c] = efc_mul(raw[2 * c + 1], scale[1]);
-    }
-    for (uint32_t k = 0; k < 4 * qd; k++) ov[2 * w + k] = efc_mul(raw[2 * w + k], scale[0]);
+    opened_from_sums(raw, w, qd, scale, ov);
 
     StageTimer t(&ctx_, "reduce rows");
     const uint32_t max_w = std::max(std::max(std::max(w, pw), aw), 4u);
@@ -262,7 +269,6 @@
         }
         return acc;
     };
-    const bool low = slab.rows == 0 && !pm && reduce_low_wanted(w + 4 * qd);
     if (!low) weights.reset();
     DevBuf<Ef> ro(&ctx_, N);
     {
@@ -326,6 +332,80 @@
     return ro;
 }
 
+DevBuf<Ef> TwoAdicFriPcs::open_reduce_one_pass(const ColMat& tr, const ColMat& chunks, unsigned log_N, Ef zeta,
+                                               Ef alpha, std::vector<Ef>& opened_values, PendingOpened* later) {
+    const unsigned log_n = log_N - fri_.log_blowup;
+    const uint64_t n = 1ull << log_n, N = 1ull << log_N;
+    const uint32_t w = tr.width, qd = chunks.width / 4;
+    TS_REQUIRE(qd <= (uint32_t)MAX_QUOTIENT_CHUNKS, TS_ERR_UNSUPPORTED, "open: more than 64 quotient chunks");
+    const Ef zeta_next = efc_mul_base(zeta, two_adic_generator(log_n));
+    const Ef pts_mont[2] = {ef_to_mont(zeta), ef_to_mont(zeta_next)};
+    const Ef scale[2] = {bary_scale(zeta, GENERATOR, n), bary_scale(zeta_next, GENERATOR, n)};
+    const size_t n_raw = 2 * (size_t)w + 4 * (size_t)qd;
+
+    const uint32_t tiles_t = bary_column_tiles(w), tiles_c = bary_column_tiles(4 * qd);
+    const size_t n_tw = 4 * (size_t)tiles_t * bary_tile_columns(w), n_cw = 4 * (size_t)tiles_c * bary_tile_columns(4 * qd);
+    const Ef am = ef_to_mont(alpha);
+    std::vector<uint32_t> cw = alpha_powers_mont(alpha, std::max(w, 4u));
+    const std::vector<uint32_t> a4(cw.begin(), cw.begin() + 16);
+    cw.resize(n_tw + n_cw, 0);
+    std::fill(cw.begin() + 4 * (size_t)w, cw.end(), 0u);
+    const Ef off_t[2] = {ef_pow(am, 0), ef_pow(am, w)};
+    for (uint32_t c = 0; c < qd; c++) {
+        const Ef off_c = ef_pow(am, 2 * (uint64_t)w + 4 * (uint64_t)c);
+        for (int k = 0; k < 4; k++) {
+            Ef ap;
+            memcpy(ap.c, &a4[4 * (size_t)k], 16);
+            const Ef wk = ef_mul(ap, off_c);
+            memcpy(&cw[n_tw + 16 * (size_t)c + 4 * k], wk.c, 16);
+        }
+    }
+    DevBuf<uint32_t> d_cw(&ctx_, cw.size());
+    h2d(ctx_, d_cw.p, cw.data(), cw.size() * 4);
+
+    DevBuf<Ef> weights(&ctx_, 2 * n), row_t(&ctx_, (size_t)tiles_t * n), row_c(&ctx_, (size_t)tiles_c * n);
+    DevBuf<Ef> d_raw(&ctx_, n_raw), d_k(&ctx_, 2);
+    Ef* const mail = reinterpret_cast<Ef*>(ctx_.mailbox(4 * n_raw));
+    if (later) {
+        ctx_.mailbox_hold(reinterpret_cast<const uint32_t*>(mail), 4 * n_raw);
+        later->ctx = &ctx_;
+        later->mail = mail;
+        later->w = w;
+        later->qd = qd;
+        later->scale[0] = scale[0];
+        later->scale[1] = scale[1];
+    }
+    {
+        StageTimer t(&ctx_, "compute opened values with Lagrange interpolation");
+        launch_bary_weights(ctx_, log_n, pts_mont, 2, weights.p, GENERATOR);
+        BaryPending pend;
+        const BaryRowSums rt{d_cw.p, row_t.p}, rc{d_cw.p + n_tw, row_c.p};
+        launch_bary_dots(ctx_, tr, log_n, weights.p, 2, d_raw.p, &pend, &rt);
+        launch_bary_dots(ctx_, chunks, log_n, weights.p, 1, d_raw.p + 2 * (size_t)w, &pend, &rc);
+        launch_bary_finish(ctx_, pend);
+        const Ef s0 = ef_to_mont(scale[0]);
+        launch_open_consts(ctx_, d_raw.p, w, 4 * qd, d_cw.p, d_cw.p + n_tw, ef_mul(s0, off_t[0]),
+                           ef_mul(ef_to_mont(scale[1]), off_t[1]), s0, mail, d_k.p);
+    }
+    DevBuf<Ef> ro(&ctx_, N);
+    {
+        StageTimer t(&ctx_, "reduce rows");
+        DevBuf<uint32_t> ro_low(&ctx_, 4 * n), ro_cols(&ctx_, 4 * N);
+        launch_reduce_low_finish(ctx_, log_n, row_t.p, tiles_t, row_c.p, tiles_c, off_t[0], off_t[1], d_k.p, weights.p,
+                                 ro_low.p);
+        coset_lde(ctx_, ro_low.p, n, 4, log_n, fri_.log_blowup, 1, ro_cols.p, N, 0, 0, false, nullptr, 0, 0,
+                  false);
+        launch_ef_interleave(ctx_, ro_cols.p, N, N, ro.p);
+    }
+    opened_values.clear();
+    if (!later) {
+        ctx_.sync();
+        opened_values.resize(n_raw);
+        opened_from_sums(mail, w, qd, scale, opened_values.data());
+    }
+    return ro;
+}
+
 void TwoAdicFriPcs::open_batch(const PcsData& d, uint64_t index, std::vector<uint32_t>& rows,
                                std::vector<uint32_t>& path) {
     TS_REQUIRE(index < (1ull << d.log_height), TS_ERR_INVALID, "open_batch: index out of range");
@@ -340,7 +420,7 @@
 void TwoAdicFriPcs::fri_prove(std::vector<DevBuf<Ef>>& inputs, const std::vector<unsigned>& log_lens,
                               BfChallenger& challenger,
                               const std::vector<const PcsData*>& input_rounds,
-                              std::vector<uint32_t>& pf, bool pass_through) {
+                              std::vector<uint32_t>& pf, bool pass_through, PendingOpened* opened_later) {
     Context& ctx = ctx_;
     const FriConfig& fri = fri_;
     TS_REQUIRE(!inputs.empty() && inputs.size() == log_lens.size(), TS_ERR_INVALID, "FRI: no input");
@@ -365,6 +445,7 @@
         fri_commit_rounds(ctx, fri, std::move(inputs[0]), 1ull << log_max_height, inputs, log_lens, 1, st);
         final_poly = fri_commit_finish(ctx, fri, challenger, st);
     }
+    if (opened_later && opened_later->active()) opened_later->fill(pf);
     std::vector<FriRound>& rounds = st.rounds;
     const uint32_t R = (uint32_t)rounds.size();
 
@@ -537,19 +618,22 @@
 
     const Ef batch_alpha = challenger.sample();
     std::vector<Ef> opened;
+    PendingOpened opened_later;
     std::vector<DevBuf<Ef>> inputs;
-    inputs.push_back(pcs.open_reduce(*trace_data, *quotient_data, zeta, batch_alpha, opened, preprocessed));
+    inputs.push_back(pcs.open_reduce(*trace_data, *quotient_data, zeta, batch_alpha, opened, preprocessed, nullptr,
+                                     &opened_later));
 
     std::vector<uint32_t> pf;
-    pf.reserve(64 + opened.size() * 4);
+    pf.reserve(64 + (opened.size() + opened_later.count()) * 4);
     ProofWriter pw(pf);
     pw.header(proof_version, st.log_degree, st.w, st.qd, air.preprocessed_width);
     pw.commitment(trace_data->root, 8);
     pw.commitment(quotient_data->root, 8);
-    pw.opened_values(opened);
+    if (opened_later.active()) pw.opened_values(opened_later);
+    else pw.opened_values(opened);
     std::vector<const PcsData*> rounds{trace_data.get(), quotient_data.get()};
     if (preprocessed) rounds.insert(rounds.begin(), preprocessed);
-    pcs.fri_prove(inputs, {st.log_N}, challenger, rounds, pf);
+    pcs.fri_prove(inputs, {st.log_N}, challenger, rounds, pf, false, &opened_later);
     return pf;
 }
 
diff --git a/tap-stark_amd/csrc/prover_common.cpp b/tap-stark_amd/csrc/prover_common.cpp
--- a/tap-stark_amd/csrc/prover_common.cpp
+++ b/tap-stark_amd/csrc/prover_common.cpp
@@ -168,6 +168,35 @@
     return opened_columns >= REDUCE_LOW_MIN_WIDTH;
 }
 
+bool open_one_pass_wanted(const Context& ctx) {
+    if (ctx.replay_mode != 0) return false;
+    if (const char* e = getenv("TS_OPEN_ONE_PASS"); e && *e) return atoi(e) != 0;
+    return true;
+}
+
+void opened_from_sums(const Ef* raw, uint32_t w, uint32_t qd, const Ef scale[2], Ef* out) {
+    for (uint32_t c = 0; c < w; c++) {
+        out[c] = efc_mul(raw[2 * c], scale[0]);
+        out[w + c] = efc_mul(raw[2 * c + 1], scale[1]);
+    }
+    for (uint32_t k = 0; k < 4 * qd; k++) out[2 * w + k] = efc_mul(raw[2 * w + k], scale[0]);
+}
+
+std::vector<Ef> PendingOpened::values() {
+    std::vector<Ef> out;
+    if (!active()) return out;
+    std::vector<Ef> raw(mail, mail + count());
+    release();
+    out.resize(raw.size());
+    opened_from_sums(raw.data(), w, qd, scale, out.data());
+    return out;
+}
+
+void PendingOpened::release() {
+    if (ctx && mail) ctx->mailbox_release();
+    mail = nullptr;
+}
+
 Statement check_statement(const FriConfig& fri, const AirProgram& air, uint32_t trace_width, uint64_t degree,
                           size_t n_public_values) {
     TS_REQUIRE(trace_width == air.width, TS_ERR_INVALID, "prove: trace width != AIR width");
@@ -240,6 +269,11 @@
 
 void ProofWriter::opened_values(const std::vector<Ef>& values) {
     for (auto& e : values) words(e.c, 4);
+}
+
+void ProofWriter::opened_values(PendingOpened& later) {
+    later.at = out_.size();
+    out_.resize(out_.size() + 4 * later.count(), 0);
 }
 
 void ProofWriter::path(std::initializer_list<Path> parts) {
diff --git a/tap-stark_amd/csrc/prover_internal.hpp b/tap-stark_amd/csrc/prover_internal.hpp
--- a/tap-stark_amd/csrc/prover_internal.hpp
+++ b/tap-stark_amd/csrc/prover_internal.hpp
@@ -49,6 +49,9 @@
 constexpr uint32_t REDUCE_LOW_MIN_WIDTH = 72;
 bool reduce_low_wanted(uint32_t opened_columns);
 
+bool open_one_pass_wanted(const Context& ctx);
+void opened_from_sums(const Ef* raw, uint32_t w, uint32_t qd, const Ef scale[2], Ef* out);
+
 struct Statement {
     unsigned log_degree, lqd;
     uint32_t qd;
@@ -77,6 +80,7 @@
     void header(uint32_t version, unsigned log_degree, uint32_t width, uint32_t qd, uint32_t extra);
     void commitment(const uint32_t* roots, size_t n_words) { words(roots, n_words); }
     void opened_values(const std::vector<Ef>& values);
+    void opened_values(PendingOpened& later);
     void begin_rounds(uint32_t n_rounds) { out_.push_back(n_rounds); }
     void begin_queries(uint32_t n_queries) { out_.push_back(n_queries); }
     void begin_input_proof(uint32_t n) { out_.push_back(n); }
```

Result: no change. 26.20 billion, median of 6 (+0.9%).
